# jiang-wenxiang/NeRFail

Hardware: AMD Instinct MI355X
Metric: rays/sec (higher is better)
Workload: dtype f32

## Files before the change

include/nerfail_hip.h:

```cpp
#ifndef NERFAIL_HIP_H
#define NERFAIL_HIP_H

#include <stddef.h>
#include <stdint.h>

#ifdef __cplusplus
extern "C" {
#endif

#define NERFAIL_ABI_VERSION 11

#define NERFAIL_OK 0
#define NERFAIL_EINVAL 1
#define NERFAIL_EHIP 2
#define NERFAIL_ENODEV 3

#define NERFAIL_RAY_FLOATS 11
#define NERFAIL_KNN 8
#define NERFAIL_MAX_DEPTH 16

int nerfail_abi_version(void);
const char* nerfail_last_error(void);
int nerfail_device_name(char* buf_host, size_t buf_len);


int nerfail_get_rays(int H, int W, const float* K4_host, const float* c2w_host,
                     float* rays_o, float* rays_d, void* stream);

int nerfail_pack_rays(const float* rays_o, const float* rays_d, int64_t n, float near_, float far_,
                      float* rays, void* stream);

int nerfail_ray_gen(int H, int W, const float* K4_host, const float* c2w_host, float near_, float far_,
                    int64_t pix_begin, int64_t pix_count, float* rays, void* stream);


int nerfail_sample_coarse(const float* rays, int64_t n_rays, const float* t_vals, int n_samples,
                          const float* t_rand, int lindisp, float* z_vals, float* pts, void* stream);

int nerfail_sample_pdf(const float* bins, const float* weights, int64_t n_rays, int n_bins,
                       const float* u, int u_is_row, int n_samples, float* samples, void* stream);

int nerfail_sample_fine(const float* rays, int64_t n_rays, const float* z_coarse, const float* weights,
                        int n_coarse, const float* u, int u_is_row, int n_fine,
                        float* z_samples, float* z_fine, float* pts, float* z_std, void* stream);


int nerfail_embed(const float* x, int64_t M, int multires, float* out, void* stream);

typedef struct nerfail_mlp_params {
    int32_t D, W;
    int32_t input_ch;
    int32_t input_ch_views;
    int32_t skip;
    int32_t reserved;
    const float* pts_w[NERFAIL_MAX_DEPTH];
    const float* pts_b[NERFAIL_MAX_DEPTH];
    const float* views_w;  const float* views_b;
    const float* feature_w; const float* feature_b;
    const float* alpha_w;  const float* alpha_b;
    const float* rgb_w;    const float* rgb_b;
} nerfail_mlp_params;

size_t nerfail_mlp_packed_floats(int D, int W, int skip);
int nerfail_mlp_pack(const nerfail_mlp_params* params_host, float* packed, void* stream);

int nerfail_mlp_fwd(const float* packed, int D, int W, int skip, const float* pts, const float* viewdirs,
                    int64_t M, int samples_per_ray, float* raw, void* stream);

int nerfail_mlp_fwd_select(int which);

int nerfail_mlp_bwd_select(int which);

int nerfail_mlp_fwd_embedded(const float* packed, int D, int W, int skip, const float* x, int64_t M,
                             float* raw, void* stream);

size_t nerfail_mlp_packed_x3_bytes(int D, int W, int skip);
int nerfail_mlp_pack_x3(const float* packed, int D, int W, int skip, void* x3, void* stream);
int nerfail_mlp_fwd_x3(const float* packed, const void* x3, int D, int W, int skip, const float* pts, const float* viewdirs,
                       int64_t M, int samples_per_ray, float* raw, void* stream);
int nerfail_mlp_fwd_embedded_x3(const float* packed, const void* x3, int D, int W, int skip, const float* x, int64_t M,
                                float* raw, void* stream);
int nerfail_mlp_fwd_rays_x3(const float* packed, const void* x3, int D, int W, int skip, const float* rays,
                            const float* z_vals, int64_t n_rays, int samples_per_ray, float* raw, float* acts, void* stream);

size_t nerfail_mlp_f16_image_bytes(int D, int W, int skip);
int nerfail_mlp_pack_f16(const nerfail_mlp_params* params_host, void* image, void* stream);
int nerfail_mlp_fwd_f16(const float* packed, const void* image, int D, int W, int skip, const float* pts,
                        const float* viewdirs, int64_t M, int samples_per_ray, float* raw, void* stream);
int nerfail_mlp_fwd_f16_train(const float* packed, const void* image, int D, int W, int skip, const float* pts,
                              const float* viewdirs, int64_t M, int samples_per_ray, float* raw, float* acts,
                              void* stream);

size_t nerfail_mlp_f16_image_T_bytes(int D, int W, int skip);
int nerfail_mlp_pack_f16_T(const nerfail_mlp_params* params_host, void* imageT, void* stream);
int nerfail_mlp_bwd_data_f16(const float* packed, const void* imageT, int D, int W, int skip, const float* d_raw,
                             const float* acts, int64_t M, float* dz, void* stream);


size_t nerfail_mlp_train_acts_floats(int D, int W, int64_t M);
size_t nerfail_mlp_train_dz_floats(int D, int W, int64_t M);
int nerfail_mlp_fwd_train(const float* packed, int D, int W, int skip, const float* pts, const float* viewdirs,
                          int64_t M, int samples_per_ray, float* raw, float* acts, void* stream);
int nerfail_mlp_fwd_rays(const float* packed, int D, int W, int skip, const float* rays, const float* z_vals,
                         int64_t n_rays, int samples_per_ray, float* raw, float* acts, void* stream);
size_t nerfail_mlp_packed_T_floats(int D, int W, int skip);
int nerfail_mlp_pack_T(const nerfail_mlp_params* params_host, float* packedT, void* stream);
int nerfail_mlp_pack_train(const nerfail_mlp_params* params_host, float* packed, float* packedT, void* stream);
int nerfail_mlp_bwd_data(const float* packed, const float* packedT, int D, int W, int skip, const float* d_raw,
                         const float* acts, int64_t M, float* dz, void* stream);
int nerfail_mlp_bwd_data2(const float* packed0, const float* packedT0, int64_t M0, const float* packed1,
                          const float* packedT1, int64_t M1, int D, int W, int skip, const float* d_raw,
                          const float* acts, float* dz, void* stream);
#define NERFAIL_DW_BF16X3 1
#define NERFAIL_DW_ACCUMULATE 2
size_t nerfail_mlp_bwd_weights_scratch_bytes(int D, int W, int skip, int64_t M0, int64_t M1, int flags);
int nerfail_mlp_bwd_weights(int D, int W, int skip, const float* acts, const float* dz, int64_t M0,
                            const nerfail_mlp_params* grads0, int64_t M1, const nerfail_mlp_params* grads1, int flags,
                            void* scratch, size_t scratch_bytes, void* stream);


int nerfail_composite(const float* raw, const float* z_vals, const float* rays, const float* noise,
                      int64_t n_rays, int n_samples, int white_bkgd,
                      float* rgb_map, float* disp_map, float* acc_map, float* weights, float* depth_map,
                      const float* pts, float* pts_max, void* stream);

int nerfail_composite_select(int which);

int nerfail_composite_bwd(const float* raw, const float* z_vals, const float* rays, const float* noise,
                          int64_t n_rays, int n_samples, int white_bkgd, const float* g_rgb_map,
                          const float* g_disp_map, const float* g_acc_map, const float* g_depth_map,
                          const float* g_weights, float* d_raw, void* stream);


int nerfail_knn8(const float* queries, int64_t n_queries, const float* points, int64_t n_points,
                 float* dist, float* idx_f32, int32_t* idx_i32, void* stream);

size_t nerfail_knn8_grid_workspace_bytes(int64_t n_points);
int nerfail_knn8_grid(const float* queries, int64_t n_queries, const float* points, int64_t n_points,
                      float* dist, float* idx_f32, int32_t* idx_i32, void* workspace, size_t workspace_bytes,
                      void* stream);
int nerfail_knn8_grid_build(const float* points, int64_t n_points, void* workspace, size_t workspace_bytes, void* stream);
int nerfail_knn8_grid_search(const float* queries, int64_t n_queries, int64_t n_points, float* dist, float* idx_f32,
                             int32_t* idx_i32, const void* workspace, size_t workspace_bytes, void* stream);
int nerfail_knn8_grid_search_view(const float* queries, int height, int width, int64_t n_points, float* dist, float* idx_f32,
                                  int32_t* idx_i32, const void* workspace, size_t workspace_bytes, void* stream);
int nerfail_knn8_grid_stats(unsigned long long* stats);


int nerfail_gauss_weight(const float* dist_and_index, int64_t B, int64_t P, float c, float* out, void* stream);

int nerfail_gauss_compose(const float* ori_img, const float* r, int64_t n_pixels, float* x_rgba, void* stream);

int nerfail_gauss_fwd(const float* spatial, int64_t Ns, const float* weight_and_index, const float* ori_img,
                      int64_t B, int64_t P, float epsilon, float* x, float* x_rgba, float* eps_minmax,
                      void* stream);

typedef struct nerfail_view_fwd {
    const float* weight_and_index;
    const void* ori_img;
} nerfail_view_fwd;
int nerfail_gauss_fwd_views(const float* spatial, int64_t Ns, const nerfail_view_fwd* views, int n_views, int64_t P,
                            int ori_is_u8, float epsilon, float* x, float* x_rgba, float* aux_alpha, unsigned char* aux_mask,
                            float* eps_minmax, void* stream);

int nerfail_gauss_bwd(const float* weight_and_index, const float* ori_img, const float* x,
                      const float* grad_x, const float* grad_x_rgba, int64_t Ns, int64_t B, int64_t P,
                      float epsilon, float* grad_spatial, void* stream);

int nerfail_fingerprint(const void* data, int64_t words_per_item, int64_t n_items, uint64_t* out, void* stream);
size_t nerfail_gauss_csr_workspace_bytes(int64_t Ns, int64_t B, int64_t P);
int nerfail_gauss_csr_build(const float* weight_and_index, int64_t Ns, int64_t B, int64_t P, int32_t* row_ptr,
                            int32_t* contrib, float* w_sorted, int32_t* row_of, void* workspace, size_t workspace_bytes,
                            void* stream);
size_t nerfail_gauss_bwd_scratch_floats(int64_t B, int64_t P, int n_rhs);
int nerfail_gauss_bwd_csr(const float* ori_img, const float* x, const float* grad_x, const float* grad_x_rgba,
                          const int32_t* row_ptr, const int32_t* contrib, const float* w_sorted, const int32_t* row_of,
                          int64_t Ns, int64_t B, int64_t P, float epsilon, float* scratch, int accumulate,
                          float* grad_spatial, void* stream);

size_t nerfail_gauss_view_pack_workspace_bytes(int64_t Ns);
int64_t nerfail_gauss_view_chunks(int64_t n_entries);
int nerfail_gauss_view_pack(const int32_t* row_ptr, const int32_t* row_of, const int32_t* contrib, int64_t Ns,
                            int64_t entry_capacity, int32_t* pos, int32_t* packed, int32_t* chunk_ord, int32_t* n_rows,
                            void* workspace, size_t workspace_bytes, void* stream);

typedef struct nerfail_view_index {
    const int32_t* packed;
    const float* w_sorted;
    const int32_t* chunk_ord;
    const int32_t* pos;
    int64_t n_entries;
    int64_t n_rows;
} nerfail_view_index;
size_t nerfail_gauss_bwd_views_scratch_floats(const nerfail_view_index* views, int n_views, int64_t P, int n_rhs);
int nerfail_gauss_bwd_views(const float* ori_img, const float* x, const float* grad_x, const float* grad_x_rgba,
                            const nerfail_view_index* views, int n_views, int64_t Ns, int64_t P, float epsilon,
                            float* scratch, float* grad_spatial, void* stream);
int nerfail_gauss_bwd_views_rgb(const float* aux_alpha, const unsigned char* aux_mask, const float* grad_x_rgba,
                                const nerfail_view_index* views, int n_views, int64_t Ns, int64_t P, float* scratch,
                                float* grad_rgb, void* stream);
int nerfail_gauss_bwd_views_rgb_step(const float* aux_alpha, const unsigned char* aux_mask, const float* grad_x_rgba,
                                     const nerfail_view_index* views, int n_views, int64_t Ns, int64_t P, float* scratch,
                                     float* grad_rgb, const float* spatial, const float* spatial_init, float a, float epsilon,
                                     int targeted, float* spatial_out, void* stream);
int nerfail_gauss_bwd_view_multi(const float* ori_img, const float* x, const float* grad_x_rgba, int n_rhs,
                                 const nerfail_view_index* view, int64_t Ns, int64_t P, float epsilon, float* scratch,
                                 float* grad_spatial, void* stream);

int nerfail_gauss_bwd_csr_multi(const float* ori_img, const float* x, const float* grad_x_rgba, int n_rhs,
                                const int32_t* row_ptr, const int32_t* contrib, const float* w_sorted, const int32_t* row_of,
                                int64_t Ns, int64_t B, int64_t P, float epsilon, float* scratch, float* grad_spatial,
                                void* stream);

size_t nerfail_deepfool_norms_scratch_bytes(int n_rhs, int64_t n);
int nerfail_deepfool_norms(const float* grads, int n_rhs, int64_t n, void* scratch, size_t scratch_bytes, float* norms2,
                           void* stream);
int nerfail_deepfool_apply(const float* grads, int n_rhs, int64_t n, const int32_t* best, const float* scale,
                           float overshoot, const float* spatial_init, float* rot, float* spatial_out, void* stream);

int nerfail_igsm_step(const float* spatial, const float* grad, const float* spatial_init, int64_t n,
                      float a, float epsilon, int targeted, float* out, void* stream);
int nerfail_igsm_step_rgb(const float* spatial, const float* grad_rgb, const float* spatial_init, int64_t n, float a,
                          float epsilon, int targeted, float* out, void* stream);

typedef struct nerfail_adam_tensor {
    float* param;
    const float* grad;
    float* exp_avg;
    float* exp_avg_sq;
    int64_t numel;
    float step_size;
    float bias_correction2_sqrt;
} nerfail_adam_tensor;
int nerfail_adam_step(const nerfail_adam_tensor* tensors, int n_tensors, double beta1, double beta2, double eps,
                      void* stream);

int nerfail_mse(const float* x, const float* y, int64_t n, float* loss, float* dx, void* stream);


size_t nerfail_cnn_packed_floats(int num_classes);
int nerfail_cnn_pack(const float* const* params_host, int num_classes, float* packed, void* stream);
size_t nerfail_cnn_workspace_bytes(int B, int H, int W, int num_classes);
size_t nerfail_cnn_mask_bytes(int B, int H, int W);
size_t nerfail_cnn_bwd_scratch_bytes(int B, int H, int W);
int nerfail_cnn_fwd(const float* packed, int num_classes, const float* x, int B, int H, int W, float* workspace,
                    unsigned char* masks, float* logits, void* stream);
int nerfail_cnn_bwd_data(const float* packed, int num_classes, const float* workspace, const unsigned char* masks,
                         const float* d_logits, int B, int H, int W, float* scratch, float* d_x, void* stream);

size_t nerfail_cnn_bwd_multi_scratch_bytes(int R, int B, int H, int W);
int nerfail_cnn_bwd_data_multi(const float* packed, int num_classes, const float* workspace, const unsigned char* masks,
                               const float* d_logits , int R, int B, int H, int W, float* scratch,
                               float* d_x , void* stream);

size_t nerfail_cnn_grad_floats(int num_classes);
size_t nerfail_cnn_bwd_weights_scratch_bytes(int B, int H, int W, int num_classes);
int nerfail_cnn_bwd_weights(const float* packed, int num_classes, const float* x, const float* workspace,
                            const unsigned char* masks, const float* d_logits, int B, int H, int W, float* scratch,
                            float* d_params, float* d_x , void* stream);

#ifdef __cplusplus
}
#endif
#endif
```

nerfail_amd/_lib.py:

```python
import ctypes
import os

import torch

_HERE = os.path.dirname(os.path.abspath(__file__))
LIB_PATH = os.environ.get('NERFAIL_HIP_LIB') or os.path.join(_HERE, 'lib', 'libnerfail_hip.so')

ABI_VERSION = 11
MAX_DEPTH = 16
DW_BF16X3, DW_ACCUMULATE = 1, 2
RAY_FLOATS = 11

c_f = ctypes.c_float
c_i = ctypes.c_int
c_i64 = ctypes.c_int64
c_p = ctypes.c_void_p


class NerfailError(RuntimeError):
    """A libnerfail_hip call returned a NERFAIL_E* code."""


class MlpParams(ctypes.Structure):
    _fields_ = [('D', ctypes.c_int32), ('W', ctypes.c_int32), ('input_ch', ctypes.c_int32),
                ('input_ch_views', ctypes.c_int32), ('skip', ctypes.c_int32), ('reserved', ctypes.c_int32),
                ('pts_w', c_p * MAX_DEPTH), ('pts_b', c_p * MAX_DEPTH),
                ('views_w', c_p), ('views_b', c_p), ('feature_w', c_p), ('feature_b', c_p),
                ('alpha_w', c_p), ('alpha_b', c_p), ('rgb_w', c_p), ('rgb_b', c_p)]


SIGNATURES = {
    'nerfail_abi_version': (c_i, []),
    'nerfail_last_error': (ctypes.c_char_p, []),
    'nerfail_device_name': (c_i, [ctypes.c_char_p, ctypes.c_size_t]),
    'nerfail_get_rays': (c_i, [c_i, c_i, c_p, c_p, c_p, c_p, c_p]),
    'nerfail_pack_rays': (c_i, [c_p, c_p, c_i64, c_f, c_f, c_p, c_p]),
    'nerfail_ray_gen': (c_i, [c_i, c_i, c_p, c_p, c_f, c_f, c_i64, c_i64, c_p, c_p]),
    'nerfail_sample_coarse': (c_i, [c_p, c_i64, c_p, c_i, c_p, c_i, c_p, c_p, c_p]),
    'nerfail_sample_pdf': (c_i, [c_p, c_p, c_i64, c_i, c_p, c_i, c_i, c_p, c_p]),
    'nerfail_sample_fine': (c_i, [c_p, c_i64, c_p, c_p, c_i, c_p, c_i, c_i, c_p, c_p, c_p, c_p, c_p]),
    'nerfail_embed': (c_i, [c_p, c_i64, c_i, c_p, c_p]),
    'nerfail_mlp_packed_floats': (ctypes.c_size_t, [c_i, c_i, c_i]),
    'nerfail_mlp_pack': (c_i, [ctypes.POINTER(MlpParams), c_p, c_p]),
    'nerfail_mlp_fwd': (c_i, [c_p, c_i, c_i, c_i, c_p, c_p, c_i64, c_i, c_p, c_p]),
    'nerfail_mlp_fwd_rays': (c_i, [c_p, c_i, c_i, c_i, c_p, c_p, c_i64, c_i, c_p, c_p, c_p]),
    'nerfail_mlp_fwd_select': (c_i, [c_i]),
    'nerfail_mlp_bwd_select': (c_i, [c_i]),
    'nerfail_mlp_fwd_embedded': (c_i, [c_p, c_i, c_i, c_i, c_p, c_i64, c_p, c_p]),
    'nerfail_mlp_packed_x3_bytes': (ctypes.c_size_t, [c_i, c_i, c_i]),
    'nerfail_mlp_pack_x3': (c_i, [c_p, c_i, c_i, c_i, c_p, c_p]),
    'nerfail_mlp_fwd_x3': (c_i, [c_p, c_p, c_i, c_i, c_i, c_p, c_p, c_i64, c_i, c_p, c_p]),
    'nerfail_mlp_fwd_embedded_x3': (c_i, [c_p, c_p, c_i, c_i, c_i, c_p, c_i64, c_p, c_p]),
    'nerfail_mlp_fwd_rays_x3': (c_i, [c_p, c_p, c_i, c_i, c_i, c_p, c_p, c_i64, c_i, c_p, c_p, c_p]),
    'nerfail_mlp_f16_image_bytes': (ctypes.c_size_t, [c_i, c_i, c_i]),
    'nerfail_mlp_pack_f16': (c_i, [ctypes.POINTER(MlpParams), c_p, c_p]),
    'nerfail_mlp_fwd_f16': (c_i, [c_p, c_p, c_i, c_i, c_i, c_p, c_p, c_i64, c_i, c_p, c_p]),
    'nerfail_mlp_fwd_f16_train': (c_i, [c_p, c_p, c_i, c_i, c_i, c_p, c_p, c_i64, c_i, c_p, c_p, c_p]),
    'nerfail_mlp_f16_image_T_bytes': (ctypes.c_size_t, [c_i, c_i, c_i]),
    'nerfail_mlp_pack_f16_T': (c_i, [ctypes.POINTER(MlpParams), c_p, c_p]),
    'nerfail_mlp_bwd_data_f16': (c_i, [c_p, c_p, c_i, c_i, c_i, c_p, c_p, c_i64, c_p, c_p]),
    'nerfail_mlp_train_acts_floats': (ctypes.c_size_t, [c_i, c_i, c_i64]),
    'nerfail_mlp_train_dz_floats': (ctypes.c_size_t, [c_i, c_i, c_i64]),
    'nerfail_mlp_fwd_train': (c_i, [c_p, c_i, c_i, c_i, c_p, c_p, c_i64, c_i, c_p, c_p, c_p]),
    'nerfail_mlp_packed_T_floats': (ctypes.c_size_t, [c_i, c_i, c_i]),
    'nerfail_mlp_pack_T': (c_i, [ctypes.POINTER(MlpParams), c_p, c_p]),
    'nerfail_mlp_pack_train': (c_i, [ctypes.POINTER(MlpParams), c_p, c_p, c_p]),
    'nerfail_mlp_bwd_data': (c_i, [c_p, c_p, c_i, c_i, c_i, c_p, c_p, c_i64, c_p, c_p]),
    'nerfail_mlp_bwd_data2': (c_i, [c_p, c_p, c_i64, c_p, c_p, c_i64, c_i, c_i, c_i, c_p, c_p, c_p, c_p]),
    'nerfail_mlp_bwd_weights_scratch_bytes': (ctypes.c_size_t, [c_i, c_i, c_i, c_i64, c_i64, c_i]),
    'nerfail_mlp_bwd_weights': (c_i, [c_i, c_i, c_i, c_p, c_p, c_i64, ctypes.POINTER(MlpParams), c_i64, ctypes.POINTER(MlpParams),
                                      c_i, c_p, ctypes.c_size_t, c_p]),
    'nerfail_composite': (c_i, [c_p, c_p, c_p, c_p, c_i64, c_i, c_i, c_p, c_p, c_p, c_p, c_p, c_p, c_p, c_p]),
    'nerfail_composite_select': (c_i, [c_i]),
    'nerfail_composite_bwd': (c_i, [c_p, c_p, c_p, c_p, c_i64, c_i, c_i, c_p, c_p, c_p, c_p, c_p, c_p, c_p]),
    'nerfail_knn8': (c_i, [c_p, c_i64, c_p, c_i64, c_p, c_p, c_p, c_p]),
    'nerfail_knn8_grid_workspace_bytes': (ctypes.c_size_t, [c_i64]),
    'nerfail_knn8_grid': (c_i, [c_p, c_i64, c_p, c_i64, c_p, c_p, c_p, c_p, ctypes.c_size_t, c_p]),
    'nerfail_knn8_grid_build': (c_i, [c_p, c_i64, c_p, ctypes.c_size_t, c_p]),
    'nerfail_knn8_grid_stats': (c_i, [c_p]),
    'nerfail_knn8_grid_search': (c_i, [c_p, c_i64, c_i64, c_p, c_p, c_p, c_p, ctypes.c_size_t, c_p]),
    'nerfail_knn8_grid_search_view': (c_i, [c_p, c_i, c_i, c_i64, c_p, c_p, c_p, c_p, ctypes.c_size_t, c_p]),
    'nerfail_gauss_weight': (c_i, [c_p, c_i64, c_i64, c_f, c_p, c_p]),
    'nerfail_gauss_compose': (c_i, [c_p, c_p, c_i64, c_p, c_p]),
    'nerfail_gauss_fwd': (c_i, [c_p, c_i64, c_p, c_p, c_i64, c_i64, c_f, c_p, c_p, c_p, c_p]),
    'nerfail_gauss_bwd': (c_i, [c_p, c_p, c_p, c_p, c_p, c_i64, c_i64, c_i64, c_f, c_p, c_p]),
    'nerfail_gauss_fwd_views': (c_i, [c_p, c_i64, c_p, c_i, c_i64, c_i, c_f, c_p, c_p, c_p, c_p, c_p, c_p]),
    'nerfail_gauss_bwd_views_rgb': (c_i, [c_p, c_p, c_p, c_p, c_i, c_i64, c_i64, c_p, c_p, c_p]),
    'nerfail_igsm_step_rgb': (c_i, [c_p, c_p, c_p, c_i64, c_f, c_f, c_i, c_p, c_p]),
    'nerfail_gauss_bwd_views_rgb_step': (c_i, [c_p, c_p, c_p, c_p, c_i, c_i64, c_i64, c_p, c_p, c_p, c_p, c_f, c_f, c_i, c_p, c_p]),
    'nerfail_fingerprint': (c_i, [c_p, c_i64, c_i64, c_p, c_p]),
    'nerfail_gauss_csr_workspace_bytes': (ctypes.c_size_t, [c_i64, c_i64, c_i64]),
    'nerfail_gauss_csr_build': (c_i, [c_p, c_i64, c_i64, c_i64, c_p, c_p, c_p, c_p, c_p, ctypes.c_size_t, c_p]),
    'nerfail_gauss_bwd_scratch_floats': (ctypes.c_size_t, [c_i64, c_i64, c_i]),
    'nerfail_gauss_view_pack_workspace_bytes': (ctypes.c_size_t, [c_i64]),
    'nerfail_gauss_view_chunks': (c_i64, [c_i64]),
    'nerfail_gauss_view_pack': (c_i, [c_p, c_p, c_p, c_i64, c_i64, c_p, c_p, c_p, c_p, c_p, ctypes.c_size_t, c_p]),
    'nerfail_gauss_bwd_view_multi': (c_i, [c_p, c_p, c_p, c_i, c_p, c_i64, c_i64, c_f, c_p, c_p, c_p]),
    'nerfail_gauss_bwd_views_scratch_floats': (ctypes.c_size_t, [c_p, c_i, c_i64, c_i]),
    'nerfail_gauss_bwd_csr': (c_i, [c_p, c_p, c_p, c_p, c_p, c_p, c_p, c_p, c_i64, c_i64, c_i64, c_f, c_p, c_i, c_p, c_p]),
    'nerfail_gauss_bwd_views': (c_i, [c_p, c_p, c_p, c_p, c_p, c_i, c_i64, c_i64, c_f, c_p, c_p, c_p]),
    'nerfail_gauss_bwd_csr_multi': (c_i, [c_p, c_p, c_p, c_i, c_p, c_p, c_p, c_p, c_i64, c_i64, c_i64, c_f, c_p, c_p, c_p]),
    'nerfail_deepfool_norms_scratch_bytes': (ctypes.c_size_t, [c_i, c_i64]),
    'nerfail_deepfool_norms': (c_i, [c_p, c_i, c_i64, c_p, ctypes.c_size_t, c_p, c_p]),
    'nerfail_deepfool_apply': (c_i, [c_p, c_i, c_i64, c_p, c_p, c_f, c_p, c_p, c_p, c_p]),
    'nerfail_igsm_step': (c_i, [c_p, c_p, c_p, c_i64, c_f, c_f, c_i, c_p, c_p]),
    'nerfail_adam_step': (c_i, [c_p, c_i, ctypes.c_double, ctypes.c_double, ctypes.c_double, c_p]),
    'nerfail_mse': (c_i, [c_p, c_p, c_i64, c_p, c_p, c_p]),
    'nerfail_cnn_packed_floats': (ctypes.c_size_t, [c_i]),
    'nerfail_cnn_pack': (c_i, [c_p, c_i, c_p, c_p]),
    'nerfail_cnn_workspace_bytes': (ctypes.c_size_t, [c_i, c_i, c_i, c_i]),
    'nerfail_cnn_mask_bytes': (ctypes.c_size_t, [c_i, c_i, c_i]),
    'nerfail_cnn_bwd_scratch_bytes': (ctypes.c_size_t, [c_i, c_i, c_i]),
    'nerfail_cnn_fwd': (c_i, [c_p, c_i, c_p, c_i, c_i, c_i, c_p, c_p, c_p, c_p]),
    'nerfail_cnn_bwd_data': (c_i, [c_p, c_i, c_p, c_p, c_p, c_i, c_i, c_i, c_p, c_p, c_p]),
    'nerfail_cnn_bwd_multi_scratch_bytes': (ctypes.c_size_t, [c_i, c_i, c_i, c_i]),
    'nerfail_cnn_bwd_data_multi': (c_i, [c_p, c_i, c_p, c_p, c_p, c_i, c_i, c_i, c_i, c_p, c_p, c_p]),
    'nerfail_cnn_grad_floats': (ctypes.c_size_t, [c_i]),
    'nerfail_cnn_bwd_weights_scratch_bytes': (ctypes.c_size_t, [c_i, c_i, c_i, c_i]),
    'nerfail_cnn_bwd_weights': (c_i, [c_p, c_i, c_p, c_p, c_p, c_p, c_i, c_i, c_i, c_p, c_p, c_p, c_p]),
}



class ViewIndexStruct(ctypes.Structure):
    _fields_ = [('packed', c_p), ('w_sorted', c_p), ('chunk_ord', c_p), ('pos', c_p), ('n_entries', c_i64), ('n_rows', c_i64)]


class ViewFwdStruct(ctypes.Structure):
    _fields_ = [('weight_and_index', c_p), ('ori_img', c_p)]


class AdamTensor(ctypes.Structure):
    _fields_ = [('param', c_p), ('grad', c_p), ('exp_avg', c_p), ('exp_avg_sq', c_p), ('numel', c_i64),
                ('step_size', c_f), ('bias_correction2_sqrt', c_f)]


_lib = None


def load():
    global _lib
    if _lib is not None:
        return _lib
    if not os.path.exists(LIB_PATH):
        raise RuntimeError('nerfail_amd: %s is missing - build it with `python -m nerfail_amd.build` '
                           '(hipcc, gfx950). There is no CPU fallback.' % LIB_PATH)
    lib = ctypes.CDLL(LIB_PATH)
    for name, (res, args) in SIGNATURES.items():
        fn = getattr(lib, name)
        fn.restype = res
        fn.argtypes = args
    v = lib.nerfail_abi_version()
    if v != ABI_VERSION:
        raise RuntimeError('nerfail_amd: ABI version %d, expected %d - rebuild the library' % (v, ABI_VERSION))
    _lib = lib
    return lib


def check(rc):
    if rc != 0:
        msg = load().nerfail_last_error().decode('utf-8', 'replace')
        raise NerfailError('libnerfail_hip error %d: %s' % (rc, msg))


def dev(t, name='tensor'):
    if t is None:
        return None
    if not isinstance(t, torch.Tensor):
        raise TypeError('%s must be a torch.Tensor' % name)
    if not t.is_cuda:
        raise RuntimeError('%s is on %s: nerfail_amd runs on the MI355X only (no CPU path)' % (name, t.device))
    if t.dtype not in (torch.float32, torch.int32, torch.uint8, torch.int64):
        raise TypeError('%s must be float32 (got %s)' % (name, t.dtype))
    if not t.is_contiguous():
        raise ValueError('%s must be contiguous' % name)
    return c_p(t.data_ptr())


def host_floats(values):
    arr = (c_f * len(values))(*[float(v) for v in values])
    return arr


def stream():
    return c_p(torch.cuda.current_stream().cuda_stream)


def f32c(t, device=None):
    t = t.detach()
    if device is not None and t.device != device:
        t = t.to(device)
    if t.dtype != torch.float32:
        t = t.float()
    return t.contiguous()


def device_name():
    buf = ctypes.create_string_buffer(256)
    check(load().nerfail_device_name(buf, 256))
    return buf.value.decode()
```

nerfail_amd/csrc/mlp.hip:

```cpp
#include <stdlib.h>
#include "mlp_layout.h"

namespace nerfail {

bool mlp_x3_covers(const MlpLayout& L, int W);
size_t mlp_x3_bytes(const MlpLayout& L, int W);
int pack_mlp_x3(const float* packed, const MlpLayout& L, int W, void* out, hipStream_t s);
int launch_mlp_x3(const MlpArgs& a, const void* img, int W, hipStream_t s);

template <int NT, bool TRAIN>
__global__ __launch_bounds__(256, 1) void nerf_mlp_fwd_kernel(MlpArgs a) {
    constexpr int OTV = NT / 2;
    const int lane = threadIdx.x & 63;
    const int wave = __builtin_amdgcn_readfirstlane(threadIdx.x >> 6);
    const int h = lane >> 5, j = lane & 31;
    const float* __restrict__ P = a.packed;
    const MlpLayout& L = a.lay;
    const long ntiles = (a.M + 31) / 32;
    const long nrounds = (ntiles + (long)gridDim.x * 4 - 1) / ((long)gridDim.x * 4);

    for (long rnd = 0; rnd < nrounds; ++rnd) {
        const long tile = (rnd * gridDim.x + blockIdx.x) * 4 + wave;
        if (tile >= ntiles) break;
        const long sraw = tile * 32 + j;
        const long s = sraw < a.M ? sraw : a.M - 1;

        float emb[4 * kEmbQuads], demb[4 * kDirQuads];
        encode_sample(a, s, h, emb, demb);

        f32x16 act[NT], acc[NT];
        float* __restrict__ A = nullptr;
        if (TRAIN) {
            A = a.acts + (size_t)tile * (train_a_slots(L.D, NT) * 1024);
            store_enc<10, 4 * kEmbQuads>(A, emb, lane);
            store_enc<4, 4 * kDirQuads>(A + 2 * 1024, demb, lane);
        }
        load_bias<NT>(acc, P + L.b_off[0], h);
        mfma_scalars<NT, kEmbQuads>(acc, P + L.w_off[0], lane, emb);
        relu_to<NT>(act, acc, true);
        if (TRAIN) {
            store_tiles<NT>(A + 3 * 1024, act, lane);
            store_mask<NT>(A + train_mask_slot0(L.D, NT) * 1024, 0, mask_of<NT>(act), lane);
        }

        float alpha = 0.f;
#pragma unroll 1
        for (int l = 1; l <= L.D; ++l) {
            if (l == L.D) {
                const float* wa = P + L.alpha_off;
                float sacc = 0.f;
#pragma unroll
                for (int t = 0; t < NT; ++t) {
                    const f32x4* p = reinterpret_cast<const f32x4*>(wa + (t * 2 + h) * 16);
#pragma unroll
                    for (int r4 = 0; r4 < 4; ++r4) {
                        const f32x4 wv = p[r4];
#pragma unroll
                        for (int e = 0; e < 4; ++e) sacc = fmaf(wv[e], act[t][4 * r4 + e], sacc);
                    }
                }
                sacc += __shfl_xor(sacc, 32, 64);
                alpha = sacc + wa[NT * 32];
            }
            load_bias<NT>(acc, P + L.b_off[l], h);
            const float* w = P + L.w_off[l];
            if (l == L.skip + 1 && L.skip >= 0) {
                if (TRAIN) {
                    float e2[4 * kEmbQuads];
                    load_enc<10, 4 * kEmbQuads>(A, e2, lane);
                    mfma_scalars<NT, kEmbQuads>(acc, w, lane, e2);
                } else {
                    mfma_scalars<NT, kEmbQuads>(acc, w, lane, emb);
                }
                w += kEmbQuads * NT * 256;
            }
            mfma_acts<NT, NT>(acc, w, lane, act);
            relu_to<NT>(act, acc, l < L.D);
            if (TRAIN) {
                store_tiles<NT>(A + (3 + l * NT) * 1024, act, lane);
                if (l < L.D) store_mask<NT>(A + train_mask_slot0(L.D, NT) * 1024, l, mask_of<NT>(act), lane);
            }
        }

        f32x16 hv[OTV];
        load_bias<OTV>(hv, P + L.b_off[L.D + 1], h);
        mfma_acts<OTV, NT>(hv, P + L.w_off[L.D + 1], lane, act);
        if (TRAIN) {
            float d2[4 * kDirQuads];
            load_enc<4, 4 * kDirQuads>(A + 2 * 1024, d2, lane);
            mfma_scalars<OTV, kDirQuads>(hv, P + L.w_off[L.D + 1] + NT * 4 * OTV * 256, lane, d2);
        } else {
            mfma_scalars<OTV, kDirQuads>(hv, P + L.w_off[L.D + 1] + NT * 4 * OTV * 256, lane, demb);
        }
        if (TRAIN) {
            f32x16 hvr[OTV];
            relu_to<OTV>(hvr, hv, true);
            store_tiles<OTV>(A + (3 + (L.D + 1) * NT) * 1024, hvr, lane);
            store_mask<OTV>(A + train_mask_slot0(L.D, NT) * 1024, L.D, mask_of<OTV>(hvr), lane);
        }

        const float* wr = P + L.rgb_off;
        float rgb[3];
#pragma unroll
        for (int c = 0; c < 3; ++c) {
            float sacc = 0.f;
#pragma unroll
            for (int t = 0; t < OTV; ++t) {
                const f32x4* p = reinterpret_cast<const f32x4*>(wr + ((c * OTV + t) * 2 + h) * 16);
#pragma unroll
                for (int r4 = 0; r4 < 4; ++r4) {
                    const f32x4 wv = p[r4];
#pragma unroll
                    for (int e = 0; e < 4; ++e) sacc = fmaf(wv[e], fmaxf(hv[t][4 * r4 + e], 0.f), sacc);
                }
            }
            sacc += __shfl_xor(sacc, 32, 64);
            rgb[c] = sacc + wr[3 * OTV * 32 + c];
        }
        if (h == 0 && sraw < a.M)
            reinterpret_cast<float4*>(a.raw)[sraw] = make_float4(rgb[0], rgb[1], rgb[2], alpha);
    }
}

static int g_fwd_select = [] {
    const char* e = getenv("NERFAIL_FWD_KERNEL");
    return e ? (e[0] == 'r' ? 1 : (e[0] == 'l' ? 2 : (e[0] == 'x' ? 3 : 0))) : 0;
}();
static bool use_lds_kernel(const MlpArgs& a) {
    if (g_fwd_select == 1) return false;
    if (g_fwd_select == 2) return true;
    return !(a.lay.D & 1) && a.lay.D <= 8;
}

static int launch_mlp(const MlpArgs& a, int W, hipStream_t s) {
    if (use_lds_kernel(a)) return launch_mlp_lds(a, W, s);
    const dim3 grid(mlp_grid_blocks((a.M + 31) / 32)), block(256);
    const bool train = a.acts != nullptr;
    switch (W) {
        case 256: if (train) nerf_mlp_fwd_kernel<8, true><<<grid, block, 0, s>>>(a); else nerf_mlp_fwd_kernel<8, false><<<grid, block, 0, s>>>(a); break;
        case 128: if (train) nerf_mlp_fwd_kernel<4, true><<<grid, block, 0, s>>>(a); else nerf_mlp_fwd_kernel<4, false><<<grid, block, 0, s>>>(a); break;
        case 64: if (train) nerf_mlp_fwd_kernel<2, true><<<grid, block, 0, s>>>(a); else nerf_mlp_fwd_kernel<2, false><<<grid, block, 0, s>>>(a); break;
        default: set_error("nerfail_mlp_fwd: unsupported W"); return NERFAIL_EINVAL;
    }
    NF_LAUNCHED("nerf_mlp_fwd_kernel");
    return NERFAIL_OK;
}

static int launch_mlp_x3_or(const MlpArgs& a, const void* img, int W, hipStream_t s) {
    if (a.acts == nullptr && (g_fwd_select == 0 || g_fwd_select == 3)) {
        if (g_fwd_select == 3 || (img != nullptr && mlp_x3_covers(a.lay, W))) {
            if (img == nullptr) { set_error("nerfail_mlp_fwd_x3: NERFAIL_FWD_KERNEL=x without a bf16x3 image"); return NERFAIL_EINVAL; }
            return launch_mlp_x3(a, img, W, s);
        }
    }
    return launch_mlp(a, W, s);
}

}

using namespace nerfail;

extern "C" int nerfail_mlp_fwd_select(int which) {
    const int prev = g_fwd_select;
    if (which >= 0 && which <= 3) g_fwd_select = which;
    return prev;
}

enum MlpInput { kInPts, kInEmbedded, kInRays };
#define MLP_REQUIRE(cond, msg) do { if (!(cond)) { set_error("%s: %s", fn, msg); return NERFAIL_EINVAL; } } while (0)
static int mlp_fwd_entry(const char* fn, MlpInput form, const float* packed, bool use_x3, const void* x3, int D, int W, int skip,
                         const float* in0, const float* in1, int64_t M, int spr, float* raw, float* acts, bool need_acts, void* stream) {
    MLP_REQUIRE(M >= 0, form == kInRays ? "n_rays is negative" : "M is negative");
    MLP_REQUIRE(form == kInEmbedded || spr >= 1, "samples_per_ray must be positive");
    MlpArgs a;
    MLP_REQUIRE(make_layout(D, W, skip, a.lay), "unsupported (D, W)");
    if (form == kInRays) M *= spr;
    if (M == 0) return NERFAIL_OK;
    MLP_REQUIRE(packed != nullptr && in0 != nullptr && (form == kInEmbedded || in1 != nullptr) && raw != nullptr &&
                (!need_acts || acts != nullptr), "NULL pointer");
    a.packed = packed; a.raw = raw; a.acts = acts; a.M = M; a.spr = form == kInEmbedded ? 1 : spr;
    a.pts = form == kInPts ? in0 : nullptr; a.viewdirs = form == kInPts ? in1 : nullptr;
    a.xemb = form == kInEmbedded ? in0 : nullptr;
    a.rays = form == kInRays ? in0 : nullptr; a.z = form == kInRays ? in1 : nullptr;
    return use_x3 ? launch_mlp_x3_or(a, x3, W, as_stream(stream)) : launch_mlp(a, W, as_stream(stream));
}
#undef MLP_REQUIRE

extern "C" int nerfail_mlp_fwd(const float* packed, int D, int W, int skip, const float* pts, const float* viewdirs,
                               int64_t M, int samples_per_ray, float* raw, void* stream) {
    return mlp_fwd_entry(__func__, kInPts, packed, false, nullptr, D, W, skip, pts, viewdirs, M, samples_per_ray, raw, nullptr, false, stream);
}

extern "C" int nerfail_mlp_fwd_embedded(const float* packed, int D, int W, int skip, const float* x, int64_t M, float* raw,
                                        void* stream) {
    return mlp_fwd_entry(__func__, kInEmbedded, packed, false, nullptr, D, W, skip, x, nullptr, M, 1, raw, nullptr, false, stream);
}

extern "C" size_t nerfail_mlp_train_acts_floats(int D, int W, int64_t M) {
    MlpLayout L;
    if (!make_layout(D, W, -1, L) || M < 0) return 0;
    return (size_t)((M + 31) / 32) * make_train_layout(D, W).a_slots * 1024;
}

extern "C" int nerfail_mlp_fwd_train(const float* packed, int D, int W, int skip, const float* pts, const float* viewdirs,
                                     int64_t M, int samples_per_ray, float* raw, float* acts, void* stream) {
    return mlp_fwd_entry(__func__, kInPts, packed, false, nullptr, D, W, skip, pts, viewdirs, M, samples_per_ray, raw, acts, true, stream);
}

extern "C" int nerfail_mlp_fwd_rays(const float* packed, int D, int W, int skip, const float* rays, const float* z_vals,
                                    int64_t n_rays, int samples_per_ray, float* raw, float* acts, void* stream) {
    return mlp_fwd_entry(__func__, kInRays, packed, false, nullptr, D, W, skip, rays, z_vals, n_rays, samples_per_ray, raw, acts, false, stream);
}

extern "C" size_t nerfail_mlp_packed_x3_bytes(int D, int W, int skip) {
    MlpLayout L;
    return make_layout(D, W, skip, L) ? mlp_x3_bytes(L, W) : 0;
}

extern "C" int nerfail_mlp_pack_x3(const float* packed, int D, int W, int skip, void* out, void* stream) {
    MlpLayout L;
    NF_REQUIRE(make_layout(D, W, skip, L), "unsupported (D, W)");
    NF_REQUIRE(packed != nullptr && out != nullptr, "NULL pointer");
    return pack_mlp_x3(packed, L, W, out, as_stream(stream));
}

extern "C" int nerfail_mlp_fwd_x3(const float* packed, const void* x3, int D, int W, int skip, const float* pts,
                                  const float* viewdirs, int64_t M, int samples_per_ray, float* raw, void* stream) {
    return mlp_fwd_entry(__func__, kInPts, packed, true, x3, D, W, skip, pts, viewdirs, M, samples_per_ray, raw, nullptr, false, stream);
}

extern "C" int nerfail_mlp_fwd_embedded_x3(const float* packed, const void* x3, int D, int W, int skip, const float* x, int64_t M,
                                           float* raw, void* stream) {
    return mlp_fwd_entry(__func__, kInEmbedded, packed, true, x3, D, W, skip, x, nullptr, M, 1, raw, nullptr, false, stream);
}

extern "C" int nerfail_mlp_fwd_rays_x3(const float* packed, const void* x3, int D, int W, int skip, const float* rays,
                                       const float* z_vals, int64_t n_rays, int samples_per_ray, float* raw, float* acts, void* stream) {
    return mlp_fwd_entry(__func__, kInRays, packed, true, x3, D, W, skip, rays, z_vals, n_rays, samples_per_ray, raw, acts, false, stream);
}
```

nerfail_amd/csrc/mlp_layout.h:

```cpp
#pragma once
#include "common.h"

namespace nerfail {

typedef float f32x16 __attribute__((ext_vector_type(16)));
typedef float f32x4 __attribute__((ext_vector_type(4)));

constexpr int kPtsCh = 63, kDirCh = 27;
constexpr int kEmbQuads = 8;
constexpr int kDirQuads = 4;

__host__ __device__ inline int enc_channel(int s, int h, int bands) {
    if (s < 3 * bands) return 3 + 6 * (s / 3) + 3 * h + (s % 3);
    if (s == 3 * bands) return h;
    if (s == 3 * bands + 1) return h ? -1 : 2;
    return -1;
}
__host__ __device__ inline int acc_channel(int r, int h) { return (r & 3) + 8 * (r >> 2) + 4 * h; }

__host__ __device__ inline int hidden_channel(int s, int h) { return 32 * (s / 16) + acc_channel(s % 16, h); }
__host__ __device__ inline int weight_column(int emb0, int h0, int dir0, int NT, int s, int h) {
    if (emb0 >= 0) {
        if (s < 4 * kEmbQuads) { const int c = enc_channel(s, h, 10); return c < 0 ? -1 : emb0 + c; }
        s -= 4 * kEmbQuads;
    }
    if (h0 >= 0) {
        if (s < 16 * NT) return h0 + hidden_channel(s, h);
        s -= 16 * NT;
    }
    if (dir0 >= 0) { const int c = enc_channel(s, h, 4); return c < 0 ? -1 : dir0 + c; }
    return -1;
}

struct MlpLayout {
    int NT, D, skip;
    unsigned w_off[NERFAIL_MAX_DEPTH + 2];
    unsigned b_off[NERFAIL_MAX_DEPTH + 2];
    unsigned w_count[NERFAIL_MAX_DEPTH + 2];
    unsigned alpha_off, rgb_off, total;
    unsigned w_total;
    unsigned stream_pad;
};
constexpr int kPiece = 256;

static inline bool layer_has_emb(int l, int skip) { return l == 0 || (skip >= 0 && l == skip + 1); }

static bool make_layout(int D, int W, int skip, MlpLayout& L) {
    if (!(W == 64 || W == 128 || W == 256)) return false;
    if (D < 2 || D > NERFAIL_MAX_DEPTH) return false;
    if (skip >= D - 1) skip = -1;
    L.NT = W / 32; L.D = D; L.skip = skip;
    const int NT = L.NT, OTV = NT / 2;
    unsigned off = 0;
    for (int l = 0; l <= D + 1; ++l) {
        const int OT = (l == D + 1) ? OTV : NT;
        int quads = 0;
        if (l <= D - 1 && layer_has_emb(l, skip)) quads += kEmbQuads;
        if (l > 0) quads += NT * 4;
        if (l == D + 1) quads += kDirQuads;
        L.w_off[l] = off; L.w_count[l] = (unsigned)quads * OT * 256; off += L.w_count[l];
    }
    const unsigned group = 4u * NT * kPiece;
    const unsigned pad = (group - off % group) % group;
    L.stream_pad = pad / kPiece; off += pad; L.w_total = off;
    for (int l = 0; l <= D + 1; ++l) { L.b_off[l] = off; off += kPiece; }
    auto up = [](unsigned n) { return (n + kPiece - 1) / kPiece * kPiece; };
    L.alpha_off = off; off += up((unsigned)NT * 32 + 4);
    L.rgb_off = off; off += up(3u * OTV * 32 + 4);
    L.total = off;
    return true;
}

struct MlpLayerDesc { const float* w; const float* b; int out_f, in_f, OT, emb0, h0, dir0; };
static inline MlpLayerDesc mlp_layer(const nerfail_mlp_params* p, const MlpLayout& L, int l) {
    const int W = 32 * L.NT;
    MlpLayerDesc d = {p->feature_w, p->feature_b, W, W, L.NT, -1, 0, -1};
    if (l < L.D) {
        const bool emb = layer_has_emb(l, L.skip);
        d.w = p->pts_w[l]; d.b = p->pts_b[l];
        d.emb0 = emb ? 0 : -1;
        d.h0 = l == 0 ? -1 : (emb ? kPtsCh : 0);
        d.in_f = (emb ? kPtsCh : 0) + (l == 0 ? 0 : W);
    } else if (l == L.D + 1) {
        d.w = p->views_w; d.b = p->views_b; d.out_f = W / 2; d.in_f = W + kDirCh; d.OT = L.NT / 2; d.dir0 = W;
    }
    return d;
}
static inline const char* mlp_layer_null_msg(const MlpLayout& L, int l) {
    return l < L.D ? "pts_linears pointer is NULL" : (l == L.D ? "feature_linear pointer is NULL" : "views_linears pointer is NULL");
}

inline int mlp_cu_count() {
    static int cus = 0;
    if (cus == 0) {
        int dev = 0, v = 0;
        if (hipGetDevice(&dev) == hipSuccess &&
            hipDeviceGetAttribute(&v, hipDeviceAttributeMultiprocessorCount, dev) == hipSuccess && v > 0) cus = v;
        else cus = 256;
    }
    return cus;
}
inline unsigned mlp_grid_blocks(long ntiles) {
    const long blocks = (ntiles + 3) / 4;
    return (unsigned)(blocks > mlp_cu_count() ? mlp_cu_count() : blocks);
}

__host__ __device__ inline int train_mask_slots(int D) { return (D + 1 + 3) / 4; }
__host__ __device__ inline int train_mask_slot0(int D, int NT) { return 3 + (D + 1) * NT + NT / 2; }
__host__ __device__ inline int train_a_slots(int D, int NT) { return train_mask_slot0(D, NT) + train_mask_slots(D); }

struct TrainLayout {
    int NT, D, OTV;
    int a_slots, a_E, a_V, a_H1, a_F, a_HV, a_MASK;
    int z_slots, z_Z0, z_ZF, z_ZV, z_ZR;
};
static inline TrainLayout make_train_layout(int D, int W) {
    TrainLayout t;
    t.NT = W / 32; t.D = D; t.OTV = t.NT / 2;
    t.a_E = 0; t.a_V = 2; t.a_H1 = 3; t.a_F = 3 + D * t.NT; t.a_HV = t.a_F + t.NT; t.a_MASK = t.a_HV + t.OTV; t.a_slots = t.a_MASK + train_mask_slots(D);
    t.z_Z0 = 0; t.z_ZF = D * t.NT; t.z_ZV = t.z_ZF + t.NT; t.z_ZR = t.z_ZV + t.OTV; t.z_slots = t.z_ZR + 1;
    return t;
}

struct MlpArgs {
    const float* packed;
    const float* pts;
    const float* viewdirs;
    const float* xemb;
    const float* rays;
    const float* z;
    float* raw;
    float* acts;
    long M;
    int spr;
    MlpLayout lay;
};
int launch_mlp_lds(const MlpArgs& a, int W, hipStream_t s);

__device__ __forceinline__ void encode_sample(const MlpArgs& a, long s, int h, float (&emb)[4 * kEmbQuads], float (&demb)[4 * kDirQuads]) {
    if (a.xemb == nullptr) {
        float px[3], vx[3];
        if (a.rays != nullptr) {
            const float* ray = a.rays + NERFAIL_RAY_FLOATS * (s / a.spr);
            const float zz = a.z[s];
#pragma unroll
            for (int d = 0; d < 3; ++d) { px[d] = mul_add_rn(ray[3 + d], zz, ray[d]); vx[d] = ray[8 + d]; }
        } else {
            const float* vd = a.viewdirs + 3 * (s / a.spr);
#pragma unroll
            for (int d = 0; d < 3; ++d) { px[d] = a.pts[3 * s + d]; vx[d] = vd[d]; }
        }
#pragma unroll
        for (int d = 0; d < 3; ++d) {
            const SinCosBands sc(px[d]);
#pragma unroll
            for (int f = 0; f < 10; ++f) emb[3 * f + d] = sc.band_sel(f, h);
        }
        emb[30] = h ? px[1] : px[0];
        emb[31] = h ? 0.f : px[2];
#pragma unroll
        for (int d = 0; d < 3; ++d) {
            const SinCosBands sc(vx[d]);
#pragma unroll
            for (int f = 0; f < 4; ++f) demb[3 * f + d] = sc.band_sel(f, h);
        }
        demb[12] = h ? vx[1] : vx[0];
        demb[13] = h ? 0.f : vx[2];
        demb[14] = 0.f; demb[15] = 0.f;
    } else {
        const float* x = a.xemb + (kPtsCh + kDirCh) * s;
#pragma unroll
        for (int st = 0; st < 4 * kEmbQuads; ++st) {
            const int c = enc_channel(st, h, 10);
            emb[st] = c >= 0 ? x[c] : 0.f;
        }
#pragma unroll
        for (int st = 0; st < 4 * kDirQuads; ++st) {
            const int c = enc_channel(st, h, 4);
            demb[st] = c >= 0 ? x[kPtsCh + c] : 0.f;
        }
    }
}

struct MlpLayoutT {
    unsigned w_off[NERFAIL_MAX_DEPTH + 2];
    unsigned total;
};
static inline void make_layout_T(int D, int NT, MlpLayoutT& L) {
    unsigned off = 0;
    L.w_off[0] = 0;
    for (int l = D + 1; l >= 1; --l) {
        L.w_off[l] = off;
        const int quads = (l == D + 1) ? (NT / 2) * 4 : NT * 4;
        off += (unsigned)quads * NT * 256;
    }
    L.total = off;
}

struct BwdArgs {
    const float* packed;
    const float* packedT;
    const float* packed2;
    const float* packedT2;
    long split;
    const float* d_raw;
    const float* acts;
    float* dz;
    long M;
    int blocks0;
    MlpLayout lay;
    MlpLayoutT layT;
    TrainLayout tl;
};
int launch_bwd_data_lds(const BwdArgs& a, int W, hipStream_t s);

template <int OT>
__device__ __forceinline__ void load_bias(f32x16 (&acc)[OT], const float* __restrict__ b, int h) {
#pragma unroll
    for (int t = 0; t < OT; ++t) {
        const f32x4* p = reinterpret_cast<const f32x4*>(b + (t * 2 + h) * 16);
        const f32x4 v0 = p[0], v1 = p[1], v2 = p[2], v3 = p[3];
        acc[t] = (f32x16){v0[0], v0[1], v0[2], v0[3], v1[0], v1[1], v1[2], v1[3],
                          v2[0], v2[1], v2[2], v2[3], v3[0], v3[1], v3[2], v3[3]};
    }
}

constexpr int kPrefetchQuads = 1;
template <int OT, int NQ, int PFQ = kPrefetchQuads, typename BSel>
__device__ __forceinline__ void mfma_part(f32x16 (&acc)[OT], const float* __restrict__ w, int lane, BSel bsel) {
    const f32x4* wp = reinterpret_cast<const f32x4*>(w) + lane;
    constexpr int PF = PFQ < NQ ? PFQ : (NQ > 1 ? NQ - 1 : 1), RING = PF + 1;
    f32x4 ring[RING][OT];
#pragma unroll
    for (int p = 0; p < PF && p < NQ; ++p)
#pragma unroll
        for (int t = 0; t < OT; ++t) ring[p][t] = wp[(p * OT + t) * 64];
#pragma unroll
    for (int q = 0; q < NQ; ++q) {
        if (q + PF < NQ) {
#pragma unroll
            for (int t = 0; t < OT; ++t)
                ring[(q + PF) % RING][t] = wp[((q + PF) * OT + t) * 64];
            __builtin_amdgcn_sched_barrier(0);
        }
#pragma unroll
        for (int e = 0; e < 4; ++e)
#pragma unroll
            for (int t = 0; t < OT; ++t)
                acc[t] = __builtin_amdgcn_mfma_f32_32x32x2f32(ring[q % RING][t][e], bsel(q, e), acc[t], 0, 0, 0);
        if (q + PF < NQ) __builtin_amdgcn_sched_barrier(0);
    }
}

template <int OT, int NQ, int PFQ = kPrefetchQuads>
__device__ __forceinline__ void mfma_scalars(f32x16 (&acc)[OT], const float* __restrict__ w, int lane,
                                             const float (&bsrc)[4 * NQ]) {
    mfma_part<OT, NQ, PFQ>(acc, w, lane, [&](int q, int e) { return bsrc[4 * q + e]; });
}

template <int OT, int NT, int PFQ = kPrefetchQuads>
__device__ __forceinline__ void mfma_acts(f32x16 (&acc)[OT], const float* __restrict__ w, int lane,
                                          const f32x16 (&in)[NT]) {
    mfma_part<OT, NT * 4, PFQ>(acc, w, lane, [&](int q, int e) { return in[q >> 2][4 * (q & 3) + e]; });
}

template <int NT>
__device__ __forceinline__ void relu_to(f32x16 (&dst)[NT], const f32x16 (&src)[NT], bool relu) {
#pragma unroll
    for (int t = 0; t < NT; ++t)
#pragma unroll
        for (int r = 0; r < 16; ++r) dst[t][r] = relu ? fmaxf(src[t][r], 0.f) : src[t][r];
}

__device__ __forceinline__ int slot_pos(int j) { return (j >> 4) * 512 + (j & 15); }
constexpr int kSlotCh = 16;

__device__ __forceinline__ int acc_lane_off(int lane) { return slot_pos(lane & 31) + (lane >> 5) * 4 * kSlotCh; }
__device__ __forceinline__ constexpr int acc_reg_off(int r) { return ((r & 3) + 8 * (r >> 2)) * kSlotCh; }

__device__ __forceinline__ void slot_store(float* p, float v) {
    __builtin_nontemporal_store(v, p);
}
template <int NTILES>
__device__ __forceinline__ void store_tiles(float* __restrict__ base, const f32x16 (&a)[NTILES], int lane) {
    float* __restrict__ lp = base + acc_lane_off(lane);
#pragma unroll
    for (int t = 0; t < NTILES; ++t)
#pragma unroll
        for (int r = 0; r < 16; ++r) slot_store(lp + t * 1024 + acc_reg_off(r), a[t][r]);
}
__device__ __forceinline__ f32x16 load_tile(const float* __restrict__ base, int lane) {
    const float* __restrict__ lp = base + acc_lane_off(lane);
    f32x16 v;
#pragma unroll
    for (int r = 0; r < 16; ++r) v[r] = lp[acc_reg_off(r)];
    return v;
}
template <int NTILES>
struct TileMask { unsigned w[(NTILES + 1) / 2]; };

__device__ __forceinline__ unsigned relu_bit(float a) {
    unsigned b;
    asm("v_med3_i32 %0, %1, 0, 1" : "=v"(b) : "v"(a));
    return b;
}
template <int NTILES>
__device__ __forceinline__ TileMask<NTILES> mask_of(const f32x16 (&a)[NTILES]) {
    TileMask<NTILES> m;
#pragma unroll
    for (int i = 0; i < (NTILES + 1) / 2; ++i) m.w[i] = 0u;
#pragma unroll
    for (int t = 0; t < NTILES; ++t)
#pragma unroll
        for (int r = 0; r < 16; ++r) m.w[t >> 1] |= relu_bit(a[t][r]) << (16 * (t & 1) + r);
    return m;
}
template <int NTILES>
__device__ __forceinline__ void store_mask(float* __restrict__ mask_slots, int entry, const TileMask<NTILES>& m, int lane) {
    unsigned* __restrict__ q = reinterpret_cast<unsigned*>(mask_slots) + entry * 256 + lane * 4;
    if constexpr (NTILES == 8) {
        *reinterpret_cast<uint4*>(q) = make_uint4(m.w[0], m.w[1], m.w[2], m.w[3]);
    } else {
#pragma unroll
        for (int i = 0; i < (NTILES + 1) / 2; ++i) q[i] = m.w[i];
    }
}
template <int NTILES>
__device__ __forceinline__ TileMask<NTILES> load_mask(const float* __restrict__ mask_slots, int entry, int lane) {
    const unsigned* __restrict__ q = reinterpret_cast<const unsigned*>(mask_slots) + entry * 256 + lane * 4;
    TileMask<NTILES> m;
    if constexpr (NTILES == 8) {
        const uint4 v = *reinterpret_cast<const uint4*>(q);
        m.w[0] = v.x; m.w[1] = v.y; m.w[2] = v.z; m.w[3] = v.w;
    } else {
#pragma unroll
        for (int i = 0; i < (NTILES + 1) / 2; ++i) m.w[i] = q[i];
    }
    return m;
}
template <int NTILES>
__device__ __forceinline__ float mask_apply(const TileMask<NTILES>& m, int t, int r, float x) {
    const int k = __builtin_amdgcn_sbfe((int)m.w[t >> 1], 16 * (t & 1) + r, 1);
    return __uint_as_float(__float_as_uint(x) & (unsigned)k);
}

__device__ __forceinline__ constexpr int enc_ch_off(int c) { return (c >> 5) * 1024 + (c & 31) * kSlotCh; }

template <int BANDS, int NSTEPS>
__device__ __forceinline__ void store_enc(float* __restrict__ base, const float (&e)[NSTEPS], int lane) {
    const int h = lane >> 5, j = lane & 31;
    float* __restrict__ lpz = base + slot_pos(j);
    float* __restrict__ lp3 = lpz + h * 3 * kSlotCh;
    float* __restrict__ lpx = lpz + (h ? enc_ch_off(32) : enc_ch_off(29));
#pragma unroll
    for (int s = 0; s < 3 * BANDS; ++s) {
        const int c0 = 3 + 6 * (s / 3) + (s % 3);
        if (c0 == 29) lpx[0] = e[s];
        else lp3[enc_ch_off(c0)] = e[s];
    }
    lpz[h * kSlotCh] = e[3 * BANDS];
    constexpr int nch = 3 + 6 * BANDS, cap = ((nch + 31) / 32) * 32;
    if (h == 0) lpz[2 * kSlotCh] = e[3 * BANDS + 1];
#pragma unroll
    for (int c = nch; c < cap; ++c)
        if (((c - nch) & 1) == h) lpz[enc_ch_off(c)] = 0.f;
}
template <int BANDS, int NSTEPS>
__device__ __forceinline__ void load_enc(const float* __restrict__ base, float (&e)[NSTEPS], int lane) {
    const int h = lane >> 5, j = lane & 31;
    const float* __restrict__ lpz = base + slot_pos(j);
    const float* __restrict__ lp3 = lpz + h * 3 * kSlotCh;
    const float* __restrict__ lpx = lpz + (h ? enc_ch_off(32) : enc_ch_off(29));
#pragma unroll
    for (int s = 0; s < 3 * BANDS; ++s) {
        const int c0 = 3 + 6 * (s / 3) + (s % 3);
        e[s] = (c0 == 29) ? lpx[0] : lp3[enc_ch_off(c0)];
    }
    e[3 * BANDS] = lpz[h * kSlotCh];
    const float z = lpz[2 * kSlotCh];
    e[3 * BANDS + 1] = h ? 0.f : z;
#pragma unroll
    for (int s = 3 * BANDS + 2; s < NSTEPS; ++s) e[s] = 0.f;
}

}
```

nerfail_amd/csrc/mlp_x3.hip:

```cpp
#include "mlp_lds.h"

namespace nerfail {

typedef __bf16 bf16x8 __attribute__((ext_vector_type(8)));
typedef __bf16 bf16x2 __attribute__((ext_vector_type(2)));
typedef unsigned u32x4 __attribute__((ext_vector_type(4)));
typedef float f32x2 __attribute__((ext_vector_type(2)));
typedef __attribute__((address_space(3))) const u32x4 lds_cu4;
typedef __attribute__((address_space(3))) const f32x2 lds_cf2;

struct X3Cfg {
    static constexpr int NT = 8;
    static constexpr int OT = 2 * NT;
    static constexpr int GP = 24;
    static constexpr int S = 4;
    static constexpr int RP = GP * S;
    static constexpr int GPW = GP / 4;
    static constexpr int SPG = GP / 3;
    static constexpr int kSync = SPG - 2;
    static constexpr int kMaxDepth = 8;
    static constexpr int kAlphaFloats = (NT * 32 + 4 + kPiece - 1) / kPiece * kPiece;
    static constexpr int kRgbFloats = (3 * (NT / 2) * 32 + 4 + kPiece - 1) / kPiece * kPiece;
    static constexpr int kConstMax = (kMaxDepth + 2) * kPiece + kAlphaFloats + kRgbFloats;
    static constexpr int kParkQuads = kEmbQuads + kDirQuads;
    static constexpr int kParkFloats = 4 * 64 * 4 * kParkQuads;
    static_assert((S - 2) * GPW <= 63, "vmcnt is a 6-bit counter");
    static_assert(GPW <= 8, "dma() covers 8 pieces per wave and group");
};

struct X3Layout {
    unsigned off[NERFAIL_MAX_DEPTH + 2];
    unsigned pieces;
};
static inline bool make_x3_layout(const MlpLayout& L, int W, X3Layout& X) {
    if (W != 256 || (L.D & 1) || L.D > X3Cfg::kMaxDepth) return false;
    unsigned off = 0;
    for (int l = 0; l <= L.D + 1; ++l) {
        const unsigned OT = (l == L.D + 1) ? L.NT / 2 : L.NT;
        const unsigned quads = L.w_count[l] / (OT * kPiece);
        if (quads & 3) return false;
        X.off[l] = off;
        off += quads / 4 * (2 * OT) * 3;
    }
    X.pieces = off;
    return off % X3Cfg::GP == 0;
}

__device__ __forceinline__ unsigned cvt_bf2(float x0, float x1) {
    return __builtin_bit_cast(unsigned, __builtin_convertvector((f32x2){x0, x1}, bf16x2));
}
__device__ __forceinline__ void sub_bf2(float& x0, float& x1, unsigned p) {
    x0 -= __uint_as_float(p << 16);
    x1 -= __uint_as_float(p & 0xffff0000u);
}

struct X3PackArgs {
    MlpLayout L;
    X3Layout X;
};
__global__ void pack_x3_kernel(const float* __restrict__ packed, X3PackArgs p, u32x4* __restrict__ img) {
    const long g = (long)blockIdx.x * blockDim.x + threadIdx.x;
    const long ts = g >> 6;
    const int lane = (int)(g & 63);
    if (ts * 3 >= p.X.pieces) return;
    int l = 0;
    while (l < p.L.D + 1 && ts * 3 >= p.X.off[l + 1]) ++l;
    const int OT32 = (l == p.L.D + 1) ? p.L.NT / 2 : p.L.NT, OT16 = 2 * OT32;
    const long r = ts - p.X.off[l] / 3;
    const int u = (int)(r / OT16), t = (int)(r % OT16);
    const int row = 16 * t + (lane & 15), lg = lane >> 4;
    const int q = 4 * u + (lg >> 1);
    const float* w = packed + p.L.w_off[l] + (row >> 5) * kPiece + ((row & 31) + 32 * (lg & 1)) * 4;
    const f32x4 q0 = *reinterpret_cast<const f32x4*>(w + (q * OT32) * kPiece);
    const f32x4 q1 = *reinterpret_cast<const f32x4*>(w + ((q + 2) * OT32) * kPiece);
    float x[8] = {q0[0], q0[1], q0[2], q0[3], q1[0], q1[1], q1[2], q1[3]};
    u32x4 hi, mid, lo;
#pragma unroll
    for (int k = 0; k < 4; ++k) {
        float a = x[2 * k], b = x[2 * k + 1];
        hi[k] = cvt_bf2(a, b);
        sub_bf2(a, b, hi[k]);
        mid[k] = cvt_bf2(a, b);
        sub_bf2(a, b, mid[k]);
        lo[k] = cvt_bf2(a, b);
    }
    u32x4* o = img + (p.X.off[l] + (long)r * 3) * 64 + lane;
    o[0] = hi;
    o[64] = mid;
    o[128] = lo;
}

struct X3Ring {
    using C = X3Cfg;
    __amdgpu_buffer_rsrc_t rsrc;
    int voff;
    float* ring;
    const float* rl;
    int total;
    int src, slot, rd, wave;
    u32x4 f1[3], f2[3];

    template <int I>
    __device__ __forceinline__ void dma_at() const {
        constexpr int B4 = I / 4;
        const int first = wave * C::GPW + 4 * B4;
        __builtin_amdgcn_raw_ptr_buffer_load_lds(rsrc, (lds_void_t*)(ring + (slot * C::GP + first) * kPiece), 16, voff,
                                                 (src + first) * (kPiece * 4), (I % 4) * kPiece * 4, 0);
    }
    __device__ __forceinline__ void dma(int i) const {
        switch (i) {
            case 0: dma_at<0>(); break;   case 1: dma_at<1>(); break;   case 2: dma_at<2>(); break;   case 3: dma_at<3>(); break;
            case 4: dma_at<4>(); break;   case 5: dma_at<5>(); break;   case 6: dma_at<6>(); break;   case 7: dma_at<7>(); break;
            default: break;
        }
    }
    __device__ __forceinline__ void group_issued() {
        src += C::GP;
        if (src >= total) src = 0;
        slot = (slot + 1 == C::S) ? 0 : slot + 1;
    }
    __device__ __forceinline__ void boundary() const {
        lds_wait_vmcnt<(C::S - 2) * C::GPW>();
        asm volatile("s_waitcnt lgkmcnt(0)" ::: "memory");
        __builtin_amdgcn_s_barrier();
        asm volatile("" ::: "memory");
    }
    __device__ __forceinline__ u32x4 frag(int POS, int p) const { return *(lds_cu4*)(rl + (rd + 3 * POS + p) * kPiece); }
    __device__ __forceinline__ void next_group() {
        rd += C::GP;
        if (rd >= C::RP) rd = 0;
    }
    __device__ __forceinline__ void start() {
#pragma unroll
        for (int g = 0; g < C::S - 1; ++g) {
#pragma unroll
            for (int i = 0; i < C::GPW; ++i) dma(i);
            group_issued();
        }
        boundary();
        dma(0);
        dma(1);
#pragma unroll
        for (int p = 0; p < 3; ++p) f1[p] = frag(0, p);
#pragma unroll
        for (int p = 0; p < 3; ++p) f2[p] = frag(1, p);
    }
};

__device__ __forceinline__ void mfma_x3(f32x4& acc, const u32x4& a, const u32x4& b) {
    acc = __builtin_amdgcn_mfma_f32_16x16x32_bf16(__builtin_bit_cast(bf16x8, a), __builtin_bit_cast(bf16x8, b), acc, 0, 0, 0);
}

__device__ __forceinline__ int x3_lane_off(int g) { return 16 * (g & 1) + 4 * (g >> 1); }
__device__ __forceinline__ int x3_tile_off(int t) { return 32 * (t >> 1) + 8 * (t & 1); }

template <int OT, int NIN>
__device__ __forceinline__ void x3_head(const f32x4 (&x)[NIN][2], const float* w, float (&out)[2]) {
    float s0 = 0.f, s1 = 0.f;
#pragma unroll
    for (int t = 0; t < OT; ++t) {
        const f32x4 wv = lds_read4(w + x3_tile_off(t));
#pragma unroll
        for (int e = 0; e < 4; ++e) {
            float v0 = x[t][0][e], v1 = x[t][1][e];
            asm("" : "+v"(v0), "+v"(v1));
            s0 = fmaf(wv[e], relu_bits(v0), s0);
            s1 = fmaf(wv[e], relu_bits(v1), s1);
        }
        __builtin_amdgcn_sched_barrier(0);
    }
    s0 += __shfl_xor(s0, 16, 64);
    s1 += __shfl_xor(s1, 16, 64);
    out[0] = s0 + __shfl_xor(s0, 32, 64);
    out[1] = s1 + __shfl_xor(s1, 32, 64);
}
template <int OT, int NIN>
__device__ __forceinline__ void x3_head3(const f32x4 (&x)[NIN][2], const float* w, int stride, float (&out)[2][3]) {
    float s[2][3] = {};
#pragma unroll
    for (int t = 0; t < OT; ++t) {
        const float* p = w + x3_tile_off(t);
        const f32x4 w0 = lds_read4(p), w1 = lds_read4(p + stride), w2 = lds_read4(p + 2 * stride);
#pragma unroll
        for (int e = 0; e < 4; ++e) {
#pragma unroll
            for (int n = 0; n < 2; ++n) {
                float v = x[t][n][e];
                asm("" : "+v"(v));
                v = relu_bits(v);
                s[n][0] = fmaf(w0[e], v, s[n][0]);
                s[n][1] = fmaf(w1[e], v, s[n][1]);
                s[n][2] = fmaf(w2[e], v, s[n][2]);
            }
        }
        __builtin_amdgcn_sched_barrier(0);
    }
#pragma unroll
    for (int n = 0; n < 2; ++n)
#pragma unroll
        for (int c = 0; c < 3; ++c) {
            const float v = s[n][c] + __shfl_xor(s[n][c], 16, 64);
            out[n][c] = v + __shfl_xor(v, 32, 64);
        }
}

template <class Side>
__device__ __forceinline__ void x3_step(X3Ring& st, const int POS, f32x4 (&acc)[2], const u32x4 (&b)[2][3], Side side) {
    using C = X3Cfg;
    const int P = (POS - C::kSync + C::SPG) % C::SPG;
    const int AHEAD = (POS + 2) % C::SPG;
    u32x4 a[3];
#pragma unroll
    for (int p = 0; p < 3; ++p) { a[p] = st.f1[p]; st.f1[p] = st.f2[p]; }
    if (P == 0) st.boundary();
#pragma unroll
    for (int k = 0; k < 12; ++k) {
        const int pr = k >> 1, n = k & 1;
        const int pa = pr == 0 || pr == 4 ? 1 : pr == 2 ? 2 : 0;
        const int pb = pr == 0 || pr == 3 ? 1 : pr == 1 ? 2 : 0;
        __builtin_amdgcn_sched_barrier(0);
        mfma_x3(acc[n], a[pa], b[n][pb]);
        __builtin_amdgcn_sched_barrier(0);
        side(k);
        if (k == 0 && P < C::GPW) st.dma(P);
        if (k == 1) st.f2[1] = st.frag(AHEAD, 1);
        if (k == 2) st.f2[0] = st.frag(AHEAD, 0);
        if (k == 3) {
            st.f2[2] = st.frag(AHEAD, 2);
            if (AHEAD == C::SPG - 1) st.next_group();
        }
    }
    if (P == C::SPG - 1) st.group_issued();
    __builtin_amdgcn_sched_barrier(0);
}

template <int OT, int NS, bool RELU, class Ld, class Hook>
__device__ __forceinline__ void x3_part(X3Ring& st, f32x4 (&out)[X3Cfg::OT][2], Ld ld, Hook hook) {
    static_assert((NS * OT) % X3Cfg::SPG == 0 && OT >= 8, "a part is a whole number of ring groups; 8 pairs per step");
    auto act = [](float v) { return RELU ? relu_bits(v) : v; };
    auto bf2_f32 = [](unsigned q) { return (f32x2){__uint_as_float(q << 16), __uint_as_float(q & 0xffff0000u)}; };
    u32x4 b[2][3];
#pragma unroll
    for (int n = 0; n < 2; ++n)
#pragma unroll
        for (int p = 0; p < 4; ++p) {
            f32x2 x = {act(ld(0, n, p, 0)), act(ld(0, n, p, 1))};
            b[n][0][p] = cvt_bf2(x[0], x[1]);
            x -= bf2_f32(b[n][0][p]);
            b[n][1][p] = cvt_bf2(x[0], x[1]);
            x -= bf2_f32(b[n][1][p]);
            b[n][2][p] = cvt_bf2(x[0], x[1]);
        }
#pragma unroll
    for (int s = 0; s < NS; ++s) {
        u32x4 bn[2][3];
        f32x2 xs[8], es[8];
#pragma unroll
        for (int t = 0; t < OT; ++t) {
            auto side = [&](int k) {
                if (s + 1 < NS && t < 8) {
                    const int n = t >> 2, p = t & 3;
                    if (k == 0) xs[t][0] = ld(s + 1, n, p, 0);
                    if (k == 1) xs[t][1] = ld(s + 1, n, p, 1);
                    if (RELU && k == 2) xs[t][0] = relu_bits(xs[t][0]);
                    if (RELU && k == 3) xs[t][1] = relu_bits(xs[t][1]);
                    if (k == 4) bn[n][0][p] = cvt_bf2(xs[t][0], xs[t][1]);
                    if (k == 5) es[t] = bf2_f32(bn[n][0][p]);
                    if (k == 6) xs[t] -= es[t];
                    if (k == 7) bn[n][1][p] = cvt_bf2(xs[t][0], xs[t][1]);
                    if (k == 8) es[t] = bf2_f32(bn[n][1][p]);
                    if (k == 9) xs[t] -= es[t];
                    if (k == 10) bn[n][2][p] = cvt_bf2(xs[t][0], xs[t][1]);
                }
                if (k >= 10) hook(s, t, k);
            };
            x3_step(st, (s * OT + t) % X3Cfg::SPG, out[t], b, side);
        }
        if (s + 1 < NS) {
#pragma unroll
            for (int n = 0; n < 2; ++n)
#pragma unroll
                for (int p = 0; p < 3; ++p) b[n][p] = bn[n][p];
        }
    }
}

template <int NT, int SKIP>
__global__ __launch_bounds__(256, 1) void nerf_mlp_fwd_x3_kernel(MlpArgs a, const void* img, int img_pieces) {
    static_assert(NT == X3Cfg::NT, "W = 256 only");
    using C = X3Cfg;
    constexpr int OT = C::OT, OTV = OT / 2;
    __shared__ __attribute__((aligned(16))) float smem[C::RP * kPiece + C::kConstMax + C::kParkFloats];
    const int tid = threadIdx.x, lane = tid & 63;
    const int wave = __builtin_amdgcn_readfirstlane(tid >> 6);
    const int h = lane >> 5, j = lane & 31;
    const int g = lane >> 4, c = lane & 15;
    const MlpLayout& L = a.lay;
    float* const ring0 = smem;
    float* const cst = smem + C::RP * kPiece;
    float* const park_w = cst + C::kConstMax + wave * (64 * 4 * C::kParkQuads);
    float* const park = park_w + lane * 4;
    const float* const park_rd = park_w + (c + 32 * (g & 1)) * 4 + (g >> 1) * 256;
    {
        const int n = (int)(L.total - L.b_off[0]);
        const float* __restrict__ gm = a.packed + L.b_off[0];
        for (int i = tid * 4; i < n; i += 1024) *reinterpret_cast<f32x4*>(cst + i) = *reinterpret_cast<const f32x4*>(gm + i);
    }
    __syncthreads();
    const float* const c_alpha = cst + (L.alpha_off - L.b_off[0]);
    const float* const c_rgb = cst + (L.rgb_off - L.b_off[0]);
    int lane_off = x3_lane_off(g);
    asm volatile("" : "+v"(lane_off));
    const float* const cst_g = cst + lane_off;

    X3Ring st;
    st.rsrc = __builtin_amdgcn_make_buffer_rsrc(const_cast<void*>(img), 0, img_pieces * (kPiece * 4), 0x00020000);
    st.voff = lane * 16; st.ring = ring0; st.rl = ring0 + lane * 4;
    st.total = img_pieces; st.src = 0; st.slot = 0; st.rd = 0; st.wave = wave;
    st.start();

    f32x4 P[OT][2], Q[OT][2];
    auto bias_tile = [&](f32x4 (&dst)[OT][2], int l, int i, int t0, int t, int k) {
        if (t == t0 && k == 10) {
            dst[i][0] = lds_read4(cst_g + l * kPiece + x3_tile_off(i));
            asm volatile("" : "+a"(dst[i][0]));
        }
        if (t == t0 + 1 && k == 11) {
            dst[i][1] = dst[i][0];
            asm volatile("" : "+a"(dst[i][1]));
        }
    };
#pragma unroll
    for (int t = 0; t < OT; ++t) { bias_tile(P, 0, t, 0, 0, 10); bias_tile(P, 0, t, 0, 1, 11); }

    const int ntiles = (int)((a.M + 31) / 32);
    const int nrounds = (int)((ntiles + (long)gridDim.x * 4 - 1) / ((long)gridDim.x * 4));
    for (int rnd = 0; rnd < nrounds; ++rnd) {
        const int tile_own = (int)(((long)rnd * gridDim.x + blockIdx.x) * 4 + wave);
        const int tile = tile_own < ntiles ? tile_own : ntiles - 1;
        int jj = j;
        asm volatile("" : "+v"(jj));
        const long sraw = (long)tile * 32 + jj;
        const long s = sraw < a.M ? sraw : a.M - 1;
        {
            float emb[4 * kEmbQuads], demb[4 * kDirQuads];
            int hh = h;
            asm volatile("" : "+v"(hh));
            encode_sample(a, s, hh, emb, demb);
#pragma unroll
            for (int k = 0; k < kEmbQuads; ++k)
                *reinterpret_cast<f32x4*>(park + k * 256) = (f32x4){emb[4 * k], emb[4 * k + 1], emb[4 * k + 2], emb[4 * k + 3]};
#pragma unroll
            for (int k = 0; k < kDirQuads; ++k)
                *reinterpret_cast<f32x4*>(park + (kEmbQuads + k) * 256) =
                    (f32x4){demb[4 * k], demb[4 * k + 1], demb[4 * k + 2], demb[4 * k + 3]};
        }
        auto b_park = [&](int q0) {
            return [=](int u, int n, int p, int e) {
                return *(__attribute__((address_space(3))) const float*)(park_rd + n * 64 + (q0 + 4 * u + 2 * (p >> 1)) * 256 + 2 * (p & 1) + e);
            };
        };
        auto b_acc = [](const f32x4 (&in)[OT][2]) {
            return [&in](int u, int n, int p, int e) { return in[2 * u + (p >> 1)][n][2 * (p & 1) + e]; };
        };
        auto no_hook = [](int, int, int) {};
        x3_part<OT, kEmbQuads / 4, false>(st, P, b_park(0), [&](int u, int t, int k) {
            for (int i = 0; i < 8; ++i) bias_tile(Q, 1, 8 * u + i, 7 + i, t, k);
        });

        float alpha[2] = {0.f, 0.f};
        auto layer = [&](f32x4 (&in)[OT][2], f32x4 (&out)[OT][2], int l, bool may_skip, bool may_be_last) __attribute__((always_inline)) {
            if (may_be_last && l == L.D) {
                x3_head<OT>(in, c_alpha + lane_off, alpha);
                alpha[0] += c_alpha[NT * 32];
                alpha[1] += c_alpha[NT * 32];
            }
            if (may_skip && l == L.skip + 1) x3_part<OT, kEmbQuads / 4, false>(st, out, b_park(0), no_hook);
            x3_part<OT, NT, true>(st, out, b_acc(in), [&](int u, int t, int k) {
                if (u > 0) { bias_tile(in, l + 1, 2 * u - 2, 8, t, k); bias_tile(in, l + 1, 2 * u - 1, 9, t, k); }
                if (u == NT - 1) { bias_tile(in, l + 1, 2 * u, 10, t, k); bias_tile(in, l + 1, 2 * u + 1, 11, t, k); }
            });
        };
#pragma unroll 1
        for (int l = 1; l < L.D; l += 2) {
            layer(P, Q, l, SKIP == 1, false);
            layer(Q, P, l + 1, SKIP == 2, true);
        }
        x3_part<OTV, NT, false>(st, Q, b_acc(P), [&](int u, int t, int k) {
            if (u > 0) { bias_tile(P, 0, 2 * u - 2, 2, t, k); bias_tile(P, 0, 2 * u - 1, 3, t, k); }
            if (u == NT - 1) { bias_tile(P, 0, 2 * u, 4, t, k); bias_tile(P, 0, 2 * u + 1, 5, t, k); }
        });
        x3_part<OTV, kDirQuads / 4, false>(st, Q, b_park(kEmbQuads), no_hook);
        float rgb[2][3];
        x3_head3<OTV>(Q, c_rgb + lane_off, OTV * 16, rgb);
        const int n = g & 1;
        int je = 16 * n + c;
        asm volatile("" : "+v"(je));
        const long sout = (long)tile * 32 + je;
        if (g < 2 && sout < a.M && tile_own < ntiles)
            reinterpret_cast<float4*>(a.raw)[sout] = make_float4((n ? rgb[1][0] : rgb[0][0]) + c_rgb[3 * OTV * 16 + 0],
                                                                 (n ? rgb[1][1] : rgb[0][1]) + c_rgb[3 * OTV * 16 + 1],
                                                                 (n ? rgb[1][2] : rgb[0][2]) + c_rgb[3 * OTV * 16 + 2],
                                                                 n ? alpha[1] : alpha[0]);
    }
    lds_wait_vmcnt<0>();
}

bool mlp_x3_covers(const MlpLayout& L, int W) {
    X3Layout X;
    return make_x3_layout(L, W, X) && L.total - L.b_off[0] <= (unsigned)X3Cfg::kConstMax;
}

size_t mlp_x3_bytes(const MlpLayout& L, int W) {
    X3Layout X;
    return mlp_x3_covers(L, W) && make_x3_layout(L, W, X) ? (size_t)X.pieces * kPiece * 4 : 0;
}

int pack_mlp_x3(const float* packed, const MlpLayout& L, int W, void* out, hipStream_t s) {
    X3PackArgs p;
    p.L = L;
    if (!mlp_x3_covers(L, W) || !make_x3_layout(L, W, p.X)) { set_error("nerfail_mlp_pack_x3: shape not covered (W = 256, even D <= 8)"); return NERFAIL_EINVAL; }
    const long threads = (long)p.X.pieces / 3 * 64;
    pack_x3_kernel<<<dim3((unsigned)((threads + 255) / 256)), dim3(256), 0, s>>>(packed, p, reinterpret_cast<u32x4*>(out));
    NF_LAUNCHED("pack_x3_kernel");
    return NERFAIL_OK;
}

int launch_mlp_x3(const MlpArgs& a, const void* img, int W, hipStream_t s) {
    X3Layout X;
    if (!mlp_x3_covers(a.lay, W) || !make_x3_layout(a.lay, W, X)) { set_error("nerf_mlp_fwd_x3_kernel: shape not covered (W = 256, even D <= 8)"); return NERFAIL_EINVAL; }
    if (a.M >= (1L << 36)) { set_error("nerfail_mlp_fwd: M must be below 2^36 samples per call"); return NERFAIL_EINVAL; }
    const dim3 grid(mlp_grid_blocks((a.M + 31) / 32)), block(256);
    const int skip_layer = a.lay.skip >= 0 ? a.lay.skip + 1 : -1;
    if (skip_layer < 0) nerf_mlp_fwd_x3_kernel<8, 0><<<grid, block, 0, s>>>(a, img, (int)X.pieces);
    else if (skip_layer & 1) nerf_mlp_fwd_x3_kernel<8, 1><<<grid, block, 0, s>>>(a, img, (int)X.pieces);
    else nerf_mlp_fwd_x3_kernel<8, 2><<<grid, block, 0, s>>>(a, img, (int)X.pieces);
    NF_LAUNCHED("nerf_mlp_fwd_x3_kernel");
    return NERFAIL_OK;
}

}
```

nerfail_amd/run_nerf.py:

```python
import os
import time

import numpy as np
import torch

from . import _lib
from .optim import Adam, decayed_lrate
from .run_nerf_helpers import (NeRF, Embedder, get_embedder, get_rays, get_rays_np, img2mse, mse2psnr, to8b,
                               sample_pdf, linspace01, _cuda, _k4, _c2w12)

np.random.seed(0)
DEBUG = False


def batchify(fn, chunk):
    if chunk is None:
        return fn

    def ret(inputs):
        return torch.cat([fn(inputs[i:i + chunk]) for i in range(0, inputs.shape[0], chunk)], 0)
    return ret


def _is_fused(embed_fn, embeddirs_fn, fn):
    return (isinstance(fn, NeRF) and isinstance(embed_fn, Embedder) and embed_fn.multires == 10 and
            isinstance(embeddirs_fn, Embedder) and embeddirs_fn.multires == 4)


def _mlp_points(fn, pts, viewdirs):
    R, N = pts.shape[0], pts.shape[1]
    raw = torch.empty((R, N, 4), dtype=torch.float32, device=pts.device)
    if getattr(fn, 'precision', 'f32') == 'f16x3':
        _lib.check(_lib.load().nerfail_mlp_fwd_f16(_lib.dev(fn.packed()), _lib.dev(fn.packed_f16()), fn.D, fn.W, fn._skip(),
                                                   _lib.dev(pts, 'pts'), _lib.dev(viewdirs, 'viewdirs'), R * N, N,
                                                   _lib.dev(raw), _lib.stream()))
        return raw
    _lib.check(_lib.load().nerfail_mlp_fwd_x3(_lib.dev(fn.packed()), _lib.dev(fn.packed_x3()), fn.D, fn.W, fn._skip(),
                                              _lib.dev(pts, 'pts'), _lib.dev(viewdirs, 'viewdirs'), R * N, N, _lib.dev(raw),
                                              _lib.stream()))
    return raw


def _mlp_rays(fn, rays, z_vals, acts=None):
    R, N = z_vals.shape
    raw = torch.empty((R, N, 4), dtype=torch.float32, device=z_vals.device)
    x3 = fn.packed_x3() if acts is None else None
    _lib.check(_lib.load().nerfail_mlp_fwd_rays_x3(_lib.dev(fn.packed()), _lib.dev(x3), fn.D, fn.W, fn._skip(),
                                                   _lib.dev(rays, 'rays'), _lib.dev(z_vals, 'z_vals'), R, N, _lib.dev(raw),
                                                   _lib.dev(acts), _lib.stream()))
    return raw


def run_network(inputs, viewdirs, fn, embed_fn, embeddirs_fn, netchunk=1024 * 64):
    dev = _cuda()
    inputs = _lib.f32c(inputs, dev)
    if viewdirs is not None and _is_fused(embed_fn, embeddirs_fn, fn) and inputs.dim() == 3:
        return _mlp_points(fn, inputs, _lib.f32c(viewdirs, dev))
    inputs_flat = torch.reshape(inputs, [-1, inputs.shape[-1]])
    embedded = embed_fn(inputs_flat)
    if viewdirs is not None:
        input_dirs = viewdirs[:, None].expand(inputs.shape)
        input_dirs_flat = torch.reshape(input_dirs, [-1, input_dirs.shape[-1]])
        embedded = torch.cat([embedded, embeddirs_fn(input_dirs_flat)], -1)
    outputs_flat = batchify(fn, netchunk)(embedded)
    return torch.reshape(outputs_flat, list(inputs.shape[:-1]) + [outputs_flat.shape[-1]])


class FusedNetworkQuery:

    def __init__(self, embed_fn, embeddirs_fn, netchunk=1024 * 64):
        self.embed_fn, self.embeddirs_fn, self.netchunk = embed_fn, embeddirs_fn, netchunk

    def __call__(self, inputs, viewdirs, network_fn):
        return run_network(inputs, viewdirs, network_fn, embed_fn=self.embed_fn, embeddirs_fn=self.embeddirs_fn,
                           netchunk=self.netchunk)


def batchify_rays(rays_flat, chunk=1024 * 32, **kwargs):
    all_ret = {}
    for i in range(0, rays_flat.shape[0], chunk):
        ret = render_rays(rays_flat[i:i + chunk], **kwargs)
        for k in ret:
            all_ret.setdefault(k, []).append(ret[k])
    return {k: (torch.cat(v, 0) if len(v) > 1 else v[0]) for k, v in all_ret.items()}


def _pack_rays(rays_o, rays_d, near, far):
    dev = _cuda()
    o = _lib.f32c(rays_o, dev).reshape(-1, 3)
    d = _lib.f32c(rays_d, dev).reshape(-1, 3)
    rays = torch.empty((o.shape[0], _lib.RAY_FLOATS), dtype=torch.float32, device=dev)
    _lib.check(_lib.load().nerfail_pack_rays(_lib.dev(o), _lib.dev(d), o.shape[0], float(near), float(far),
                                             _lib.dev(rays), _lib.stream()))
    return rays


def ray_gen(H, W, K, c2w, near, far, pix_begin=0, pix_count=None):
    dev = _cuda()
    n = H * W - pix_begin if pix_count is None else pix_count
    rays = torch.empty((n, _lib.RAY_FLOATS), dtype=torch.float32, device=dev)
    _lib.check(_lib.load().nerfail_ray_gen(int(H), int(W), _k4(K), _c2w12(c2w), float(near), float(far),
                                           int(pix_begin), int(n), _lib.dev(rays), _lib.stream()))
    return rays


def _render(H, W, K, chunk, rays, c2w, ndc, near, far, use_viewdirs, c2w_staticcam, want_pts_max, kwargs):
    if ndc:
        raise NotImplementedError('ndc=True is LLFF-only (RN:112-114); the blender configs pass ndc=False')
    if not use_viewdirs:
        raise NotImplementedError('HIP path implements use_viewdirs=True (all configs/*.txt)')
    if c2w is not None:
        if c2w_staticcam is not None:
            rays_flat = ray_gen(H, W, K, c2w_staticcam, near, far)
            rays_flat[:, 8:11] = ray_gen(H, W, K, c2w, near, far)[:, 8:11]
        else:
            rays_flat = ray_gen(H, W, K, c2w, near, far)
        sh = (H, W, 3)
    else:
        rays_o, rays_d = rays
        sh = tuple(rays_d.shape)
        rays_flat = _pack_rays(rays_o, rays_d, near, far)
    all_ret = batchify_rays(rays_flat, chunk, want_pts_max=want_pts_max, **kwargs)
    for k in all_ret:
        all_ret[k] = torch.reshape(all_ret[k], list(sh[:-1]) + list(all_ret[k].shape[1:]))
    k_extract = ['rgb_map', 'disp_map', 'acc_map'] + (['pts_max'] if want_pts_max else [])
    ret_list = [all_ret[k] for k in k_extract]
    ret_dict = {k: all_ret[k] for k in all_ret if k not in k_extract}
    return ret_list + [ret_dict]


def render(H, W, K, chunk=1024 * 32, rays=None, c2w=None, ndc=True, near=0., far=1., use_viewdirs=False,
           c2w_staticcam=None, **kwargs):
    return _render(H, W, K, chunk, rays, c2w, ndc, near, far, use_viewdirs, c2w_staticcam, False, kwargs)


def render_path(render_poses, hwf, K, chunk, render_kwargs, gt_imgs=None, savedir=None, render_factor=0):
    H, W, focal = hwf
    if render_factor != 0:
        H, W, focal = H // render_factor, W // render_factor, focal / render_factor
    rgbs, disps = [], []
    t = time.time()
    for i, c2w in enumerate(render_poses):
        print(i, time.time() - t)
        t = time.time()
        rgb, disp, acc, _ = render(H, W, K, chunk=chunk, c2w=c2w[:3, :4], **render_kwargs)
        rgbs.append(rgb.cpu().numpy())
        disps.append(disp.cpu().numpy())
        if savedir is not None:
            import imageio
            imageio.imwrite(os.path.join(savedir, '{:03d}.png'.format(i)), to8b(rgbs[-1]))
    return np.stack(rgbs, 0), np.stack(disps, 0)


def create_nerf(args):
    dev = _cuda()
    embed_fn, input_ch = get_embedder(args.multires, args.i_embed)
    input_ch_views, embeddirs_fn = 0, None
    if args.use_viewdirs:
        embeddirs_fn, input_ch_views = get_embedder(args.multires_views, args.i_embed)
    output_ch = 5 if args.N_importance > 0 else 4
    skips = [4]
    model = NeRF(D=args.netdepth, W=args.netwidth, input_ch=input_ch, output_ch=output_ch, skips=skips,
                 input_ch_views=input_ch_views, use_viewdirs=args.use_viewdirs).to(dev)
    grad_vars = list(model.parameters())
    model_fine = None
    if args.N_importance > 0:
        model_fine = NeRF(D=args.netdepth_fine, W=args.netwidth_fine, input_ch=input_ch, output_ch=output_ch,
                          skips=skips, input_ch_views=input_ch_views, use_viewdirs=args.use_viewdirs).to(dev)
        grad_vars += list(model_fine.parameters())
    network_query_fn = FusedNetworkQuery(embed_fn, embeddirs_fn, args.netchunk)
    optimizer = Adam(params=grad_vars, lr=args.lrate, betas=(0.9, 0.999))
    start = 0
    basedir, expname = args.basedir, args.expname
    if getattr(args, 'ft_path', None) is not None and args.ft_path != 'None':
        ckpts = [args.ft_path]
    else:
        d = os.path.join(basedir, expname)
        ckpts = [os.path.join(d, f) for f in sorted(os.listdir(d)) if 'tar' in f] if os.path.isdir(d) else []
    print('Found ckpts', ckpts)
    if len(ckpts) > 0 and not args.no_reload:
        ckpt = torch.load(ckpts[-1], map_location=dev)
        start = ckpt['global_step']
        optimizer.load_state_dict(ckpt['optimizer_state_dict'])
        model.load_state_dict(ckpt['network_fn_state_dict'])
        if model_fine is not None:
            model_fine.load_state_dict(ckpt['network_fine_state_dict'])
    render_kwargs_train = {
        'network_query_fn': network_query_fn, 'perturb': args.perturb, 'N_importance': args.N_importance,
        'network_fine': model_fine, 'N_samples': args.N_samples, 'network_fn': model,
        'use_viewdirs': args.use_viewdirs, 'white_bkgd': args.white_bkgd, 'raw_noise_std': args.raw_noise_std,
    }
    if args.dataset_type != 'llff' or args.no_ndc:
        render_kwargs_train['ndc'] = False
        render_kwargs_train['lindisp'] = args.lindisp
    render_kwargs_test = {k: render_kwargs_train[k] for k in render_kwargs_train}
    render_kwargs_test['perturb'] = False
    render_kwargs_test['raw_noise_std'] = 0.
    return render_kwargs_train, render_kwargs_test, start, grad_vars, optimizer


def _composite(raw, z_vals, rays, noise, white_bkgd, pts=None, want_pts_max=None):
    R, N = z_vals.shape
    dev = raw.device
    if want_pts_max is None:
        want_pts_max = pts is not None
    rgb_map = torch.empty((R, 3), dtype=torch.float32, device=dev)
    disp_map = torch.empty((R,), dtype=torch.float32, device=dev)
    acc_map = torch.empty((R,), dtype=torch.float32, device=dev)
    weights = torch.empty((R, N), dtype=torch.float32, device=dev)
    depth_map = torch.empty((R,), dtype=torch.float32, device=dev)
    pts_max = torch.empty((R, 3), dtype=torch.float32, device=dev) if want_pts_max else None
    _lib.check(_lib.load().nerfail_composite(
        _lib.dev(raw, 'raw'), _lib.dev(z_vals, 'z_vals'), _lib.dev(rays, 'rays'), _lib.dev(noise, 'noise'), R, N,
        int(bool(white_bkgd)), _lib.dev(rgb_map), _lib.dev(disp_map), _lib.dev(acc_map), _lib.dev(weights),
        _lib.dev(depth_map), _lib.dev(pts, 'pts') if want_pts_max else None, _lib.dev(pts_max), _lib.stream()))
    return rgb_map, disp_map, acc_map, weights, depth_map, pts_max


def _noise(shape, raw_noise_std, pytest, noise, dev):
    if noise is not None:
        return _lib.f32c(noise, dev).reshape(shape)
    if raw_noise_std > 0.:
        if pytest:
            np.random.seed(0)
            return torch.Tensor(np.random.rand(*shape) * raw_noise_std).to(dev).contiguous()
        return (torch.randn(shape, device=dev) * raw_noise_std).contiguous()
    return None


def raw2outputs(raw, z_vals, rays_d, raw_noise_std=0, white_bkgd=False, pytest=False, noise=None):
    dev = _cuda()
    raw_in = raw
    raw, z_vals, rays_d = _lib.f32c(raw, dev), _lib.f32c(z_vals, dev), _lib.f32c(rays_d, dev)
    R = z_vals.shape[0]
    rays = torch.zeros((R, _lib.RAY_FLOATS), dtype=torch.float32, device=dev)
    rays[:, 3:6] = rays_d
    nz = _noise(tuple(z_vals.shape), raw_noise_std, pytest, noise, dev)
    if nz is None:
        from . import ops
        raw_g = raw_in.to(dev).float().contiguous() if isinstance(raw_in, torch.Tensor) and raw_in.requires_grad else raw
        return tuple(torch.ops.nerfail_mi.composite(raw_g, z_vals, rays, bool(white_bkgd)))
    return _composite(raw, z_vals, rays, nz, white_bkgd)[:5]


def render_rays(ray_batch, network_fn, network_query_fn, N_samples, retraw=False, lindisp=False, perturb=0.,
                N_importance=0, network_fine=None, white_bkgd=False, raw_noise_std=0., verbose=False, pytest=False,
                want_pts_max=False, t_rand=None, u=None, noise=None, noise_fine=None):
    dev = _cuda()
    rays = _lib.f32c(ray_batch, dev)
    if rays.shape[-1] != _lib.RAY_FLOATS:
        raise NotImplementedError('ray_batch must be [R, 11] (use_viewdirs=True packing, RN:116-123)')
    R = rays.shape[0]
    q = network_query_fn
    fused = q is None or (isinstance(q, FusedNetworkQuery) and _is_fused(q.embed_fn, q.embeddirs_fn, network_fn))

    if perturb > 0. and t_rand is None:
        if pytest:
            np.random.seed(0)
            t_rand = torch.Tensor(np.random.rand(R, N_samples))
        else:
            t_rand = torch.rand((R, N_samples), device=dev)
    t_rand = _lib.f32c(t_rand, dev) if perturb > 0. else None
    if N_importance > 0 and u is None:
        det = (perturb == 0.)
        if pytest:
            np.random.seed(0)
            u = torch.Tensor(np.linspace(0., 1., N_importance)) if det else torch.Tensor(np.random.rand(R, N_importance))
        else:
            u = linspace01(N_importance, dev) if det else torch.rand((R, N_importance), device=dev)
    if u is not None:
        u = _lib.f32c(u, dev)
    nz = _noise((R, N_samples), raw_noise_std, pytest, noise, dev)
    nzf = _noise((R, N_samples + N_importance), raw_noise_std, pytest, noise_fine, dev) if N_importance > 0 else None

    def pipeline(rays, train=False):
        return _render_rays_pipeline(rays, network_fn, network_fine, q if not fused else None, N_samples, N_importance,
                                     lindisp, white_bkgd, t_rand, u, nz, nzf, want_pts_max, train)

    needs_grad = fused and torch.is_grad_enabled() and any(
        p.requires_grad for n in (network_fn, network_fine) if n is not None for p in n.parameters())
    if needs_grad:
        from . import _train
        nets = [network_fn] + ([network_fine] if network_fine is not None else [])
        params = [p for n in nets for p in _train.ordered_params(n)]
        cfg = dict(pipeline=pipeline, network_fn=network_fn, network_fine=network_fine, white_bkgd=white_bkgd,
                   retraw=retraw)
        o = _train.RenderRaysTrain.apply(rays, cfg, *params)
        out = dict(zip(('rgb_map', 'disp_map', 'acc_map', 'rgb0', 'disp0', 'acc0', 'z_std', 'pts_max', 'raw'), o))
    else:
        out = pipeline(rays, False)

    ret = {'rgb_map': out['rgb_map'], 'disp_map': out['disp_map'], 'acc_map': out['acc_map']}
    if want_pts_max:
        ret['pts_max'] = out['pts_max']
    if retraw:
        ret['raw'] = out['raw']
    if N_importance > 0:
        ret.update(rgb0=out['rgb0'], disp0=out['disp0'], acc0=out['acc0'], z_std=out['z_std'])
    if DEBUG:
        for k in ret:
            if torch.isnan(ret[k]).any() or torch.isinf(ret[k]).any():
                print(f"! [Numerical Error] {k} contains nan or inf.")
    return ret


def _render_rays_pipeline(rays, network_fn, network_fine, user_query, N_samples, N_importance, lindisp, white_bkgd,
                          t_rand, u, nz, nzf, want_pts_max, train):
    dev = rays.device
    lib = _lib.load()
    R = rays.shape[0]
    st = _lib.stream()
    viewdirs = rays[:, 8:11].contiguous()

    def empty():
        return torch.empty((0,), dtype=torch.float32, device=dev)

    def wants_pts(fn):
        return user_query is not None or getattr(fn, 'precision', 'f32') == 'f16x3'

    def query(p, z, fn):
        if user_query is not None:
            return _lib.f32c(user_query(p, viewdirs, fn), dev), None
        if train:
            from . import _train
            a_ = acts_for.pop(0) if acts_for else None
            if p is None:
                return _train.mlp_fwd_train_rays(fn, rays, z, acts=a_)
            return _train.mlp_fwd_train(fn, p, viewdirs, acts=a_)
        if p is None:
            return _mlp_rays(fn, rays, z), None
        return _mlp_points(fn, p, viewdirs), None

    acts_all, acts_for = None, []
    if train and user_query is None and N_importance > 0:
        from . import _train
        run_fn_ = network_fn if network_fine is None else network_fine
        if _train._same_arch(network_fn, run_fn_) and (R * N_samples) % 32 == 0:
            nc, nf = _train.acts_floats(network_fn, R * N_samples), _train.acts_floats(run_fn_, R * (N_samples + N_importance))
            acts_all = torch.empty((nc + nf,), dtype=torch.float32, device=dev)
            acts_for = [acts_all[:nc], acts_all[nc:]]

    z_vals = torch.empty((R, N_samples), dtype=torch.float32, device=dev)
    pts = torch.empty((R, N_samples, 3), dtype=torch.float32, device=dev) if wants_pts(network_fn) else None
    t_lin = linspace01(N_samples, dev)
    _lib.check(lib.nerfail_sample_coarse(_lib.dev(rays), R, _lib.dev(t_lin), int(N_samples),
                                         _lib.dev(t_rand, 't_rand'), int(bool(lindisp)), _lib.dev(z_vals), _lib.dev(pts), st))
    raw, acts = query(pts, z_vals, network_fn)
    last_pass = not (N_importance > 0)
    rgb_map, disp_map, acc_map, weights, depth_map, pts_max = _composite(
        raw, z_vals, rays, nz, white_bkgd, pts, want_pts_max and last_pass)
    out = {'rgb0': empty(), 'disp0': empty(), 'acc0': empty(), 'z_std': empty()}
    saved = {'rays': rays, 'coarse': dict(raw=raw, z=z_vals, acts=acts, noise=nz), 'fine': None, 'acts_all': acts_all}
    if N_importance > 0:
        out.update(rgb0=rgb_map, disp0=disp_map, acc0=acc_map)
        Nt = N_samples + N_importance
        z_samples = torch.empty((R, N_importance), dtype=torch.float32, device=dev)
        z_fine = torch.empty((R, Nt), dtype=torch.float32, device=dev)
        run_fn = network_fn if network_fine is None else network_fine
        pts = torch.empty((R, Nt, 3), dtype=torch.float32, device=dev) if wants_pts(run_fn) else None
        z_std = torch.empty((R,), dtype=torch.float32, device=dev)
        _lib.check(lib.nerfail_sample_fine(_lib.dev(rays), R, _lib.dev(z_vals), _lib.dev(weights), int(N_samples),
                                           _lib.dev(u, 'u'), int(u.dim() == 1), int(N_importance), _lib.dev(z_samples),
                                           _lib.dev(z_fine), _lib.dev(pts), _lib.dev(z_std), st))
        z_vals = z_fine
        raw, acts = query(pts, z_vals, run_fn)
        rgb_map, disp_map, acc_map, weights, depth_map, pts_max = _composite(
            raw, z_vals, rays, nzf, white_bkgd, pts, want_pts_max)
        out['z_std'] = z_std
        saved['fine'] = dict(raw=raw, z=z_vals, acts=acts, noise=nzf)
    out.update(rgb_map=rgb_map, disp_map=disp_map, acc_map=acc_map, raw=raw,
               pts_max=pts_max if pts_max is not None else empty())
    if train:
        out['_saved'] = saved
    return out
```

nerfail_amd/run_nerf_helpers.py:

```python
import numpy as np
import torch
import torch.nn as nn

from . import _lib

class _Img2Mse(torch.autograd.Function):

    @staticmethod
    def forward(ctx, x, y):
        xc, yc = _lib.f32c(x), _lib.f32c(y)
        loss = torch.empty((), dtype=torch.float32, device=x.device)
        dx = torch.empty_like(xc) if x.requires_grad else None
        _lib.check(_lib.load().nerfail_mse(_lib.dev(xc), _lib.dev(yc), xc.numel(), _lib.dev(loss), _lib.dev(dx), _lib.stream()))
        ctx.dx = dx
        return loss

    @staticmethod
    def backward(ctx, g):
        return (None if ctx.dx is None else ctx.dx * g), None


MSE_FUSED_MAX = 1 << 16


def img2mse(x, y):
    if (isinstance(x, torch.Tensor) and isinstance(y, torch.Tensor) and x.is_cuda and y.is_cuda and x.dtype == torch.float32
            and y.dtype == torch.float32 and x.shape == y.shape and not y.requires_grad and 0 < x.numel() <= MSE_FUSED_MAX):
        return _Img2Mse.apply(x, y)
    return torch.mean((x - y) ** 2)


mse2psnr = lambda x: -10. * torch.log(x) / torch.log(torch.Tensor([10.]).to(x.device))
to8b = lambda x: (255 * np.clip(x, 0, 1)).astype(np.uint8)


def _cuda():
    if not torch.cuda.is_available():
        raise RuntimeError('nerfail_amd needs an MI355X (torch.cuda.is_available() is False); no CPU path exists')
    return torch.device('cuda', torch.cuda.current_device())


class Embedder:

    def __init__(self, multires):
        self.multires = int(multires)
        self.out_dim = 3 + 6 * self.multires

    def embed(self, inputs):
        x = _lib.f32c(inputs, _cuda())
        assert x.shape[-1] == 3, 'input_dims is 3 (RH:58)'
        flat = x.reshape(-1, 3)
        out = torch.empty((flat.shape[0], self.out_dim), dtype=torch.float32, device=x.device)
        _lib.check(_lib.load().nerfail_embed(_lib.dev(flat, 'inputs'), flat.shape[0], self.multires,
                                             _lib.dev(out), _lib.stream()))
        return out.reshape(x.shape[:-1] + (self.out_dim,))

    __call__ = embed


def get_embedder(multires, i=0, device=None):
    if i == -1:
        return nn.Identity(), 3
    eo = Embedder(multires)
    return eo, eo.out_dim


class NeRF(nn.Module):

    def __init__(self, D=8, W=256, input_ch=3, input_ch_views=3, output_ch=4, skips=[4], use_viewdirs=False):
        super(NeRF, self).__init__()
        self.D = D
        self.W = W
        self.input_ch = input_ch
        self.input_ch_views = input_ch_views
        self.skips = skips
        self.use_viewdirs = use_viewdirs
        self.pts_linears = nn.ModuleList(
            [nn.Linear(input_ch, W)] + [nn.Linear(W, W) if i not in self.skips else nn.Linear(W + input_ch, W)
                                        for i in range(D - 1)])
        self.views_linears = nn.ModuleList([nn.Linear(input_ch_views + W, W // 2)])
        if use_viewdirs:
            self.feature_linear = nn.Linear(W, W)
            self.alpha_linear = nn.Linear(W, 1)
            self.rgb_linear = nn.Linear(W // 2, 3)
        else:
            self.output_linear = nn.Linear(W, output_ch)
        self._packed = None
        self._packed_key = None
        self._packed16 = None
        self._packed16_key = None
        self._packed_x3 = None
        self._packed_x3_key = None
        self.precision = 'f32'

    def _skip(self):
        s = [i for i in self.skips if i < self.D - 1]
        if len(s) > 1:
            raise NotImplementedError('one skip connection supported (the reference always uses skips=[4])')
        return s[0] if s else -1

    def packed(self):
        if not self.use_viewdirs:
            raise NotImplementedError('HIP path implements use_viewdirs=True (all NeRFail configs, configs/*.txt)')
        params = list(self.parameters())
        if not params[0].is_cuda:
            raise RuntimeError('NeRF parameters are on %s: call .cuda() - there is no CPU path' % params[0].device)
        key = tuple((p.data_ptr(), p._version) for p in params)
        if self._packed is not None and key == self._packed_key:
            return self._packed
        lib = _lib.load()
        n = lib.nerfail_mlp_packed_floats(self.D, self.W, self._skip())
        if n == 0:
            raise NotImplementedError('unsupported NeRF shape D=%d W=%d (W in {64,128,256})' % (self.D, self.W))
        keep = []
        mp = self._mlp_params(keep)
        buf = torch.empty((n,), dtype=torch.float32, device=params[0].device)
        _lib.check(lib.nerfail_mlp_pack(mp, _lib.dev(buf), _lib.stream()))
        self._packed, self._packed_key = buf, key
        return buf

    def packed_x3(self):
        f32 = self.packed()
        params = list(self.parameters())
        key = tuple((p.data_ptr(), p._version) for p in params)
        if self._packed_x3_key == key:
            return self._packed_x3
        lib = _lib.load()
        n = lib.nerfail_mlp_packed_x3_bytes(self.D, self.W, self._skip())
        buf = None
        if n:
            buf = torch.empty((n,), dtype=torch.uint8, device=f32.device)
            _lib.check(lib.nerfail_mlp_pack_x3(_lib.dev(f32), self.D, self.W, self._skip(), _lib.dev(buf), _lib.stream()))
        self._packed_x3, self._packed_x3_key = buf, key
        return buf

    def _mlp_params(self, keep):
        mp = _lib.MlpParams()
        mp.D, mp.W, mp.input_ch, mp.input_ch_views, mp.skip = self.D, self.W, self.input_ch, self.input_ch_views, self._skip()

        def ptr(t):
            t = _lib.f32c(t)
            keep.append(t)
            return t.data_ptr()
        for i, l in enumerate(self.pts_linears):
            mp.pts_w[i] = ptr(l.weight)
            mp.pts_b[i] = ptr(l.bias)
        mp.views_w, mp.views_b = ptr(self.views_linears[0].weight), ptr(self.views_linears[0].bias)
        mp.feature_w, mp.feature_b = ptr(self.feature_linear.weight), ptr(self.feature_linear.bias)
        mp.alpha_w, mp.alpha_b = ptr(self.alpha_linear.weight), ptr(self.alpha_linear.bias)
        mp.rgb_w, mp.rgb_b = ptr(self.rgb_linear.weight), ptr(self.rgb_linear.bias)
        return mp

    def packed_f16(self):
        params = list(self.parameters())
        key = tuple((p.data_ptr(), p._version) for p in params)
        self._f16_poll()
        if self._packed16 is not None and key == self._packed16_key:
            return self._packed16
        lib = _lib.load()
        n = lib.nerfail_mlp_f16_image_bytes(self.D, self.W, self._skip())
        if n == 0:
            raise NotImplementedError('unsupported NeRF shape D=%d W=%d' % (self.D, self.W))
        self.check_f16x3_range()
        keep = []
        mp = self._mlp_params(keep)
        buf = torch.empty((n,), dtype=torch.uint8, device=params[0].device)
        _lib.check(lib.nerfail_mlp_pack_f16(mp, _lib.dev(buf), _lib.stream()))
        self._packed16, self._packed16_key = buf, key
        return buf

    F16X3_MAX_WEIGHT = 60.0

    def check_f16x3_range(self, sync=False):
        self._f16_poll()
        ws = [p.detach() for n_, p in self.named_parameters() if n_.endswith('weight')]
        with torch.no_grad():
            m = torch.stack(torch._foreach_norm(ws, float('inf'))).max()
        if sync or not m.is_cuda or not getattr(self, '_f16_checked_once', False):
            self._f16_checked_once = True
            self._f16_verdict(float(m))
            return
        self._f16_poll(wait=True)
        host = getattr(self, '_f16_host', None)
        if host is None:
            host = self._f16_host = torch.empty((1,), dtype=torch.float32).pin_memory()
        host.copy_(m.reshape(1), non_blocking=True)
        ev = torch.cuda.Event()
        ev.record()
        self._f16_pending = ev

    def _f16_poll(self, wait=False):
        ev = getattr(self, '_f16_pending', None)
        if ev is None:
            return
        if wait:
            ev.synchronize()
        if ev.query():
            self._f16_pending = None
            self._f16_verdict(float(self._f16_host[0]))

    def _f16_verdict(self, m):
        if not m < self.F16X3_MAX_WEIGHT:
            raise ValueError("NeRF.precision = 'f16x3': max |weight| = %g is outside the range of the split-precision kernels "
                             "(|w| < %g); use precision = 'f32'" % (m, self.F16X3_MAX_WEIGHT))

    def forward(self, x):
        x = _lib.f32c(x, _cuda())
        assert x.shape[-1] == self.input_ch + self.input_ch_views
        flat = x.reshape(-1, x.shape[-1])
        out = torch.empty((flat.shape[0], 4), dtype=torch.float32, device=flat.device)
        _lib.check(_lib.load().nerfail_mlp_fwd_embedded_x3(_lib.dev(self.packed()), _lib.dev(self.packed_x3()), self.D, self.W,
                                                           self._skip(), _lib.dev(flat, 'x'), flat.shape[0], _lib.dev(out),
                                                           _lib.stream()))
        return out.reshape(x.shape[:-1] + (4,))


def _k4(K):
    return _lib.host_floats([K[0][0], K[1][1], K[0][2], K[1][2]])


def _c2w12(c2w):
    c = torch.as_tensor(c2w).detach().to('cpu', torch.float32)[:3, :4].reshape(-1).tolist()
    return _lib.host_floats(c)


def get_rays(H, W, K, c2w):
    dev = _cuda()
    rays_o = torch.empty((H, W, 3), dtype=torch.float32, device=dev)
    rays_d = torch.empty((H, W, 3), dtype=torch.float32, device=dev)
    _lib.check(_lib.load().nerfail_get_rays(int(H), int(W), _k4(K), _c2w12(c2w), _lib.dev(rays_o), _lib.dev(rays_d),
                                            _lib.stream()))
    return rays_o, rays_d


def get_rays_np(H, W, K, c2w):
    o, d = get_rays(H, W, K, c2w)
    return o.cpu().numpy(), d.cpu().numpy()


def ndc_rays(H, W, focal, near, rays_o, rays_d):
    raise NotImplementedError('ndc_rays (RH:179-196) is LLFF-only; every NeRFail config sets ndc=False (RN:250-252)')


_LINSPACE = {}


def linspace01(n, device):
    key = (int(n), str(device))
    if key not in _LINSPACE:
        _LINSPACE[key] = torch.linspace(0., 1., steps=int(n)).to(device)
    return _LINSPACE[key]


def sample_pdf(bins, weights, N_samples, det=False, pytest=False, u=None):
    dev = _cuda()
    bins = _lib.f32c(bins, dev)
    weights = _lib.f32c(weights, dev)
    lead = bins.shape[:-1]
    nb = bins.shape[-1]
    assert weights.shape[-1] == nb - 1
    b2, w2 = bins.reshape(-1, nb), weights.reshape(-1, nb - 1)
    R = b2.shape[0]
    if pytest:
        np.random.seed(0)
        if det:
            u = torch.Tensor(np.linspace(0., 1., N_samples)).to(dev)
        else:
            u = torch.Tensor(np.random.rand(*(list(lead) + [N_samples]))).to(dev)
    elif u is None:
        u = linspace01(N_samples, dev) if det else torch.rand(list(lead) + [N_samples], device=dev)
    u = _lib.f32c(u, dev)
    is_row = int(u.dim() == 1)
    if not is_row:
        u = u.reshape(R, N_samples)
    from . import ops
    out = torch.ops.nerfail_mi.sample_pdf(b2, w2, u)
    return out.reshape(tuple(lead) + (N_samples,))
```

Before: 917,700.

## Fold feature linear layer into view layer weights for x3 forward kernel

```diff
diff --git a/include/nerfail_hip.h b/include/nerfail_hip.h
--- a/include/nerfail_hip.h
+++ b/include/nerfail_hip.h
@@ -8,7 +8,7 @@
 extern "C" {
 #endif
 
-#define NERFAIL_ABI_VERSION 11
+#define NERFAIL_ABI_VERSION 12
 
 #define NERFAIL_OK 0
 #define NERFAIL_EINVAL 1
@@ -82,6 +82,16 @@
                                 float* raw, void* stream);
 int nerfail_mlp_fwd_rays_x3(const float* packed, const void* x3, int D, int W, int skip, const float* rays,
                             const float* z_vals, int64_t n_rays, int samples_per_ray, float* raw, float* acts, void* stream);
+
+size_t nerfail_mlp_packed_x3f_bytes(int D, int W, int skip);
+size_t nerfail_mlp_x3f_composed_floats(int D, int W, int skip);
+int nerfail_mlp_pack_x3f(const float* packed, int D, int W, int skip, void* x3f, void* stream);
+int nerfail_mlp_fwd_x3f(const float* packed, const void* x3f, int D, int W, int skip, const float* pts, const float* viewdirs,
+                        int64_t M, int samples_per_ray, float* raw, void* stream);
+int nerfail_mlp_fwd_embedded_x3f(const float* packed, const void* x3f, int D, int W, int skip, const float* x, int64_t M,
+                                 float* raw, void* stream);
+int nerfail_mlp_fwd_rays_x3f(const float* packed, const void* x3f, int D, int W, int skip, const float* rays,
+                             const float* z_vals, int64_t n_rays, int samples_per_ray, float* raw, float* acts, void* stream);
 
 size_t nerfail_mlp_f16_image_bytes(int D, int W, int skip);
 int nerfail_mlp_pack_f16(const nerfail_mlp_params* params_host, void* image, void* stream);
diff --git a/nerfail_amd/_lib.py b/nerfail_amd/_lib.py
--- a/nerfail_amd/_lib.py
+++ b/nerfail_amd/_lib.py
@@ -6,7 +6,7 @@
 _HERE = os.path.dirname(os.path.abspath(__file__))
 LIB_PATH = os.environ.get('NERFAIL_HIP_LIB') or os.path.join(_HERE, 'lib', 'libnerfail_hip.so')
 
-ABI_VERSION = 11
+ABI_VERSION = 12
 MAX_DEPTH = 16
 DW_BF16X3, DW_ACCUMULATE = 1, 2
 RAY_FLOATS = 11
@@ -52,6 +52,12 @@
     'nerfail_mlp_fwd_x3': (c_i, [c_p, c_p, c_i, c_i, c_i, c_p, c_p, c_i64, c_i, c_p, c_p]),
     'nerfail_mlp_fwd_embedded_x3': (c_i, [c_p, c_p, c_i, c_i, c_i, c_p, c_i64, c_p, c_p]),
     'nerfail_mlp_fwd_rays_x3': (c_i, [c_p, c_p, c_i, c_i, c_i, c_p, c_p, c_i64, c_i, c_p, c_p, c_p]),
+    'nerfail_mlp_packed_x3f_bytes': (ctypes.c_size_t, [c_i, c_i, c_i]),
+    'nerfail_mlp_x3f_composed_floats': (ctypes.c_size_t, [c_i, c_i, c_i]),
+    'nerfail_mlp_pack_x3f': (c_i, [c_p, c_i, c_i, c_i, c_p, c_p]),
+    'nerfail_mlp_fwd_x3f': (c_i, [c_p, c_p, c_i, c_i, c_i, c_p, c_p, c_i64, c_i, c_p, c_p]),
+    'nerfail_mlp_fwd_embedded_x3f': (c_i, [c_p, c_p, c_i, c_i, c_i, c_p, c_i64, c_p, c_p]),
+    'nerfail_mlp_fwd_rays_x3f': (c_i, [c_p, c_p, c_i, c_i, c_i, c_p, c_p, c_i64, c_i, c_p, c_p, c_p]),
     'nerfail_mlp_f16_image_bytes': (ctypes.c_size_t, [c_i, c_i, c_i]),
     'nerfail_mlp_pack_f16': (c_i, [ctypes.POINTER(MlpParams), c_p, c_p]),
     'nerfail_mlp_fwd_f16': (c_i, [c_p, c_p, c_i, c_i, c_i, c_p, c_p, c_i64, c_i, c_p, c_p]),
diff --git a/nerfail_amd/csrc/mlp.hip b/nerfail_amd/csrc/mlp.hip
--- a/nerfail_amd/csrc/mlp.hip
+++ b/nerfail_amd/csrc/mlp.hip
@@ -6,7 +6,10 @@
 bool mlp_x3_covers(const MlpLayout& L, int W);
 size_t mlp_x3_bytes(const MlpLayout& L, int W);
 int pack_mlp_x3(const float* packed, const MlpLayout& L, int W, void* out, hipStream_t s);
-int launch_mlp_x3(const MlpArgs& a, const void* img, int W, hipStream_t s);
+int launch_mlp_x3(const MlpArgs& a, const void* img, int W, bool fold, hipStream_t s);
+size_t mlp_x3f_bytes(const MlpLayout& L, int W);
+size_t mlp_x3f_composed_floats(const MlpLayout& L, int W);
+int pack_mlp_x3f(const float* packed, const MlpLayout& L, int W, void* out, hipStream_t s);
 
 template <int NT, bool TRAIN>
 __global__ __launch_bounds__(256, 1) void nerf_mlp_fwd_kernel(MlpArgs a) {
@@ -146,11 +149,11 @@
     return NERFAIL_OK;
 }
 
-static int launch_mlp_x3_or(const MlpArgs& a, const void* img, int W, hipStream_t s) {
+static int launch_mlp_x3_or(const char* fn, const MlpArgs& a, const void* img, int W, bool fold, hipStream_t s) {
     if (a.acts == nullptr && (g_fwd_select == 0 || g_fwd_select == 3)) {
         if (g_fwd_select == 3 || (img != nullptr && mlp_x3_covers(a.lay, W))) {
-            if (img == nullptr) { set_error("nerfail_mlp_fwd_x3: NERFAIL_FWD_KERNEL=x without a bf16x3 image"); return NERFAIL_EINVAL; }
-            return launch_mlp_x3(a, img, W, s);
+            if (img == nullptr) { set_error("%s: NERFAIL_FWD_KERNEL=x without a bf16x3 image", fn); return NERFAIL_EINVAL; }
+            return launch_mlp_x3(a, img, W, fold, s);
         }
     }
     return launch_mlp(a, W, s);
@@ -167,8 +170,9 @@
 }
 
 enum MlpInput { kInPts, kInEmbedded, kInRays };
+enum MlpSel { kF32, kX3, kX3Fold };
 #define MLP_REQUIRE(cond, msg) do { if (!(cond)) { set_error("%s: %s", fn, msg); return NERFAIL_EINVAL; } } while (0)
-static int mlp_fwd_entry(const char* fn, MlpInput form, const float* packed, bool use_x3, const void* x3, int D, int W, int skip,
+static int mlp_fwd_entry(const char* fn, MlpInput form, const float* packed, MlpSel sel, const void* x3, int D, int W, int skip,
                          const float* in0, const float* in1, int64_t M, int spr, float* raw, float* acts, bool need_acts, void* stream) {
     MLP_REQUIRE(M >= 0, form == kInRays ? "n_rays is negative" : "M is negative");
     MLP_REQUIRE(form == kInEmbedded || spr >= 1, "samples_per_ray must be positive");
@@ -182,18 +186,18 @@
     a.pts = form == kInPts ? in0 : nullptr; a.viewdirs = form == kInPts ? in1 : nullptr;
     a.xemb = form == kInEmbedded ? in0 : nullptr;
     a.rays = form == kInRays ? in0 : nullptr; a.z = form == kInRays ? in1 : nullptr;
-    return use_x3 ? launch_mlp_x3_or(a, x3, W, as_stream(stream)) : launch_mlp(a, W, as_stream(stream));
+    return sel != kF32 ? launch_mlp_x3_or(fn, a, x3, W, sel == kX3Fold, as_stream(stream)) : launch_mlp(a, W, as_stream(stream));
 }
 #undef MLP_REQUIRE
 
 extern "C" int nerfail_mlp_fwd(const float* packed, int D, int W, int skip, const float* pts, const float* viewdirs,
                                int64_t M, int samples_per_ray, float* raw, void* stream) {
-    return mlp_fwd_entry(__func__, kInPts, packed, false, nullptr, D, W, skip, pts, viewdirs, M, samples_per_ray, raw, nullptr, false, stream);
+    return mlp_fwd_entry(__func__, kInPts, packed, kF32, nullptr, D, W, skip, pts, viewdirs, M, samples_per_ray, raw, nullptr, false, stream);
 }
 
 extern "C" int nerfail_mlp_fwd_embedded(const float* packed, int D, int W, int skip, const float* x, int64_t M, float* raw,
                                         void* stream) {
-    return mlp_fwd_entry(__func__, kInEmbedded, packed, false, nullptr, D, W, skip, x, nullptr, M, 1, raw, nullptr, false, stream);
+    return mlp_fwd_entry(__func__, kInEmbedded, packed, kF32, nullptr, D, W, skip, x, nullptr, M, 1, raw, nullptr, false, stream);
 }
 
 extern "C" size_t nerfail_mlp_train_acts_floats(int D, int W, int64_t M) {
@@ -204,12 +208,12 @@
 
 extern "C" int nerfail_mlp_fwd_train(const float* packed, int D, int W, int skip, const float* pts, const float* viewdirs,
                                      int64_t M, int samples_per_ray, float* raw, float* acts, void* stream) {
-    return mlp_fwd_entry(__func__, kInPts, packed, false, nullptr, D, W, skip, pts, viewdirs, M, samples_per_ray, raw, acts, true, stream);
+    return mlp_fwd_entry(__func__, kInPts, packed, kF32, nullptr, D, W, skip, pts, viewdirs, M, samples_per_ray, raw, acts, true, stream);
 }
 
 extern "C" int nerfail_mlp_fwd_rays(const float* packed, int D, int W, int skip, const float* rays, const float* z_vals,
                                     int64_t n_rays, int samples_per_ray, float* raw, float* acts, void* stream) {
-    return mlp_fwd_entry(__func__, kInRays, packed, false, nullptr, D, W, skip, rays, z_vals, n_rays, samples_per_ray, raw, acts, false, stream);
+    return mlp_fwd_entry(__func__, kInRays, packed, kF32, nullptr, D, W, skip, rays, z_vals, n_rays, samples_per_ray, raw, acts, false, stream);
 }
 
 extern "C" size_t nerfail_mlp_packed_x3_bytes(int D, int W, int skip) {
@@ -226,15 +230,47 @@
 
 extern "C" int nerfail_mlp_fwd_x3(const float* packed, const void* x3, int D, int W, int skip, const float* pts,
                                   const float* viewdirs, int64_t M, int samples_per_ray, float* raw, void* stream) {
-    return mlp_fwd_entry(__func__, kInPts, packed, true, x3, D, W, skip, pts, viewdirs, M, samples_per_ray, raw, nullptr, false, stream);
+    return mlp_fwd_entry(__func__, kInPts, packed, kX3, x3, D, W, skip, pts, viewdirs, M, samples_per_ray, raw, nullptr, false, stream);
 }
 
 extern "C" int nerfail_mlp_fwd_embedded_x3(const float* packed, const void* x3, int D, int W, int skip, const float* x, int64_t M,
                                            float* raw, void* stream) {
-    return mlp_fwd_entry(__func__, kInEmbedded, packed, true, x3, D, W, skip, x, nullptr, M, 1, raw, nullptr, false, stream);
+    return mlp_fwd_entry(__func__, kInEmbedded, packed, kX3, x3, D, W, skip, x, nullptr, M, 1, raw, nullptr, false, stream);
 }
 
 extern "C" int nerfail_mlp_fwd_rays_x3(const float* packed, const void* x3, int D, int W, int skip, const float* rays,
                                        const float* z_vals, int64_t n_rays, int samples_per_ray, float* raw, float* acts, void* stream) {
-    return mlp_fwd_entry(__func__, kInRays, packed, true, x3, D, W, skip, rays, z_vals, n_rays, samples_per_ray, raw, acts, false, stream);
-}
+    return mlp_fwd_entry(__func__, kInRays, packed, kX3, x3, D, W, skip, rays, z_vals, n_rays, samples_per_ray, raw, acts, false, stream);
+}
+
+extern "C" size_t nerfail_mlp_packed_x3f_bytes(int D, int W, int skip) {
+    MlpLayout L;
+    return make_layout(D, W, skip, L) ? mlp_x3f_bytes(L, W) : 0;
+}
+
+extern "C" size_t nerfail_mlp_x3f_composed_floats(int D, int W, int skip) {
+    MlpLayout L;
+    return make_layout(D, W, skip, L) ? mlp_x3f_composed_floats(L, W) : 0;
+}
+
+extern "C" int nerfail_mlp_pack_x3f(const float* packed, int D, int W, int skip, void* out, void* stream) {
+    MlpLayout L;
+    NF_REQUIRE(make_layout(D, W, skip, L), "unsupported (D, W)");
+    NF_REQUIRE(packed != nullptr && out != nullptr, "NULL pointer");
+    return pack_mlp_x3f(packed, L, W, out, as_stream(stream));
+}
+
+extern "C" int nerfail_mlp_fwd_x3f(const float* packed, const void* x3f, int D, int W, int skip, const float* pts,
+                                   const float* viewdirs, int64_t M, int samples_per_ray, float* raw, void* stream) {
+    return mlp_fwd_entry(__func__, kInPts, packed, kX3Fold, x3f, D, W, skip, pts, viewdirs, M, samples_per_ray, raw, nullptr, false, stream);
+}
+
+extern "C" int nerfail_mlp_fwd_embedded_x3f(const float* packed, const void* x3f, int D, int W, int skip, const float* x, int64_t M,
+                                            float* raw, void* stream) {
+    return mlp_fwd_entry(__func__, kInEmbedded, packed, kX3Fold, x3f, D, W, skip, x, nullptr, M, 1, raw, nullptr, false, stream);
+}
+
+extern "C" int nerfail_mlp_fwd_rays_x3f(const float* packed, const void* x3f, int D, int W, int skip, const float* rays,
+                                        const float* z_vals, int64_t n_rays, int samples_per_ray, float* raw, float* acts, void* stream) {
+    return mlp_fwd_entry(__func__, kInRays, packed, kX3Fold, x3f, D, W, skip, rays, z_vals, n_rays, samples_per_ray, raw, acts, false, stream);
+}
diff --git a/nerfail_amd/csrc/mlp_layout.h b/nerfail_amd/csrc/mlp_layout.h
--- a/nerfail_amd/csrc/mlp_layout.h
+++ b/nerfail_amd/csrc/mlp_layout.h
@@ -16,9 +16,19 @@
     if (s == 3 * bands + 1) return h ? -1 : 2;
     return -1;
 }
-__host__ __device__ inline int acc_channel(int r, int h) { return (r & 3) + 8 * (r >> 2) + 4 * h; }
-
-__host__ __device__ inline int hidden_channel(int s, int h) { return 32 * (s / 16) + acc_channel(s % 16, h); }
+__host__ __device__ constexpr int acc_channel(int r, int h) { return (r & 3) + 8 * (r >> 2) + 4 * h; }
+
+__host__ __device__ constexpr int hidden_channel(int s, int h) { return 32 * (s / 16) + acc_channel(s % 16, h); }
+__host__ __device__ constexpr int hidden_half(int c) { return (c >> 2) & 1; }
+__host__ __device__ constexpr int hidden_step(int c) { return 16 * (c >> 5) + (c & 3) + 4 * ((c & 31) >> 3); }
+__host__ __device__ constexpr int bias_index(int c) { return 32 * (c >> 5) + 16 * hidden_half(c) + (hidden_step(c) & 15); }
+constexpr bool hidden_inverse_holds() {
+    for (int c = 0; c < 256; ++c)
+        if (hidden_channel(hidden_step(c), hidden_half(c)) != c || hidden_step(c) >= 128 || bias_index(c) >= 256 ||
+            32 * (bias_index(c) >> 5) + acc_channel(bias_index(c) & 15, (bias_index(c) >> 4) & 1) != c) return false;
+    return true;
+}
+static_assert(hidden_inverse_holds(), "hidden_step / hidden_half / bias_index invert hidden_channel / the bias order");
 __host__ __device__ inline int weight_column(int emb0, int h0, int dir0, int NT, int s, int h) {
     if (emb0 >= 0) {
         if (s < 4 * kEmbQuads) { const int c = enc_channel(s, h, 10); return c < 0 ? -1 : emb0 + c; }
diff --git a/nerfail_amd/csrc/mlp_x3.hip b/nerfail_amd/csrc/mlp_x3.hip
--- a/nerfail_amd/csrc/mlp_x3.hip
+++ b/nerfail_amd/csrc/mlp_x3.hip
@@ -45,6 +45,15 @@
     X.pieces = off;
     return off % X3Cfg::GP == 0;
 }
+static inline bool make_x3f_layout(const MlpLayout& L, int W, X3Layout& X) {
+    if (!make_x3_layout(L, W, X)) return false;
+    const unsigned feature = X.off[L.D + 1] - X.off[L.D];
+    X.off[L.D + 1] = X.off[L.D];
+    X.pieces -= feature;
+    return X.pieces % X3Cfg::GP == 0;
+}
+__host__ __device__ inline unsigned x3f_const_floats(const MlpLayout& L) { return L.total - L.b_off[0]; }
+static inline unsigned x3f_composed_floats(const MlpLayout& L) { return (unsigned)(L.NT / 2 * 32) * (L.NT * 32) + kPiece; }
 
 __device__ __forceinline__ unsigned cvt_bf2(float x0, float x1) {
     return __builtin_bit_cast(unsigned, __builtin_convertvector((f32x2){x0, x1}, bf16x2));
@@ -58,7 +67,8 @@
     MlpLayout L;
     X3Layout X;
 };
-__global__ void pack_x3_kernel(const float* __restrict__ packed, X3PackArgs p, u32x4* __restrict__ img) {
+template <bool FOLD>
+__global__ void pack_x3_kernel(const float* __restrict__ packed, X3PackArgs p, u32x4* __restrict__ img, const float* __restrict__ wc) {
     const long g = (long)blockIdx.x * blockDim.x + threadIdx.x;
     const long ts = g >> 6;
     const int lane = (int)(g & 63);
@@ -74,6 +84,10 @@
     const f32x4 q0 = *reinterpret_cast<const f32x4*>(w + (q * OT32) * kPiece);
     const f32x4 q1 = *reinterpret_cast<const f32x4*>(w + ((q + 2) * OT32) * kPiece);
     float x[8] = {q0[0], q0[1], q0[2], q0[3], q1[0], q1[1], q1[2], q1[3]};
+    if (FOLD && l == p.L.D + 1 && u < p.L.NT) {
+#pragma unroll
+        for (int j = 0; j < 8; ++j) x[j] = wc[row * (32 * p.L.NT) + 32 * u + 4 * lg + (j & 3) + 16 * (j >> 2)];
+    }
     u32x4 hi, mid, lo;
 #pragma unroll
     for (int k = 0; k < 4; ++k) {
@@ -88,6 +102,39 @@
     o[0] = hi;
     o[64] = mid;
     o[128] = lo;
+}
+
+__device__ __forceinline__ float x3f_weight(const float* __restrict__ packed, const MlpLayout& L, int l, int OT32, int i, int c) {
+    const int s = hidden_step(c), h = hidden_half(c);
+    return packed[L.w_off[l] + ((s >> 2) * OT32 + (i >> 5)) * kPiece + ((i & 31) + 32 * h) * 4 + (s & 3)];
+}
+__global__ void compose_x3f_kernel(const float* __restrict__ packed, MlpLayout L, float* __restrict__ cst, float* __restrict__ comp) {
+    const int W = 32 * L.NT, WV = W / 2, D = L.D;
+    const int nconst = (int)x3f_const_floats(L);
+    int t = (int)(blockIdx.x * blockDim.x + threadIdx.x);
+    if (t < WV * W) {
+        const int i = t / W, j = t % W;
+        double acc = 0.;
+        for (int m = 0; m < W; ++m)
+            acc += (double)x3f_weight(packed, L, D + 1, L.NT / 2, i, m) * (double)x3f_weight(packed, L, D, L.NT, m, j);
+        comp[t] = (float)acc;
+        return;
+    }
+    t -= WV * W;
+    if (t >= nconst + kPiece) return;
+    const int pos = t < nconst ? t % kPiece : t - nconst;
+    const bool in_bias = t < nconst && t / kPiece == D;
+    if (t < nconst && !in_bias) { cst[t] = packed[L.b_off[0] + t]; return; }
+    const int ch = in_bias ? 32 * (pos >> 5) + acc_channel(pos & 15, (pos >> 4) & 1) : pos;
+    float v = 0.f;
+    if (ch < WV && pos < (in_bias ? W : WV)) {
+        double acc = 0.;
+        for (int m = 0; m < W; ++m)
+            acc += (double)x3f_weight(packed, L, D + 1, L.NT / 2, ch, m) * (double)packed[L.b_off[D] + bias_index(m)];
+        acc += (double)packed[L.b_off[D + 1] + bias_index(ch)];
+        v = (float)acc;
+    }
+    (t < nconst ? cst[t] : comp[WV * W + pos]) = v;
 }
 
 struct X3Ring {
@@ -285,7 +332,7 @@
     }
 }
 
-template <int NT, int SKIP>
+template <int NT, int SKIP, bool FOLD>
 __global__ __launch_bounds__(256, 1) void nerf_mlp_fwd_x3_kernel(MlpArgs a, const void* img, int img_pieces) {
     static_assert(NT == X3Cfg::NT, "W = 256 only");
     using C = X3Cfg;
@@ -303,7 +350,7 @@
     const float* const park_rd = park_w + (c + 32 * (g & 1)) * 4 + (g >> 1) * 256;
     {
         const int n = (int)(L.total - L.b_off[0]);
-        const float* __restrict__ gm = a.packed + L.b_off[0];
+        const float* __restrict__ gm = FOLD ? static_cast<const float*>(img) + (long)img_pieces * kPiece : a.packed + L.b_off[0];
         for (int i = tid * 4; i < n; i += 1024) *reinterpret_cast<f32x4*>(cst + i) = *reinterpret_cast<const f32x4*>(gm + i);
     }
     __syncthreads();
@@ -346,7 +393,13 @@
             float emb[4 * kEmbQuads], demb[4 * kDirQuads];
             int hh = h;
             asm volatile("" : "+v"(hh));
-            encode_sample(a, s, hh, emb, demb);
+            if constexpr (FOLD) {
+                MlpArgs ar = a;
+                asm volatile("" : "+s"(ar.spr));
+                encode_sample(ar, s, hh, emb, demb);
+            } else {
+                encode_sample(a, s, hh, emb, demb);
+            }
 #pragma unroll
             for (int k = 0; k < kEmbQuads; ++k)
                 *reinterpret_cast<f32x4*>(park + k * 256) = (f32x4){emb[4 * k], emb[4 * k + 1], emb[4 * k + 2], emb[4 * k + 3]};
@@ -370,29 +423,44 @@
 
         float alpha[2] = {0.f, 0.f};
         auto layer = [&](f32x4 (&in)[OT][2], f32x4 (&out)[OT][2], int l, bool may_skip, bool may_be_last) __attribute__((always_inline)) {
-            if (may_be_last && l == L.D) {
+            if (!FOLD && may_be_last && l == L.D) {
                 x3_head<OT>(in, c_alpha + lane_off, alpha);
                 alpha[0] += c_alpha[NT * 32];
                 alpha[1] += c_alpha[NT * 32];
             }
             if (may_skip && l == L.skip + 1) x3_part<OT, kEmbQuads / 4, false>(st, out, b_park(0), no_hook);
+            int lb = l + 1;
+            if constexpr (FOLD) asm volatile("" : "+s"(lb));
             x3_part<OT, NT, true>(st, out, b_acc(in), [&](int u, int t, int k) {
-                if (u > 0) { bias_tile(in, l + 1, 2 * u - 2, 8, t, k); bias_tile(in, l + 1, 2 * u - 1, 9, t, k); }
-                if (u == NT - 1) { bias_tile(in, l + 1, 2 * u, 10, t, k); bias_tile(in, l + 1, 2 * u + 1, 11, t, k); }
+                if (u > 0) { bias_tile(in, lb, 2 * u - 2, 8, t, k); bias_tile(in, lb, 2 * u - 1, 9, t, k); }
+                if (u == NT - 1) { bias_tile(in, lb, 2 * u, 10, t, k); bias_tile(in, lb, 2 * u + 1, 11, t, k); }
             });
+            if (FOLD && may_be_last && l == L.D - 1) {
+                x3_head<OT>(out, c_alpha + lane_off, alpha);
+                alpha[0] += c_alpha[NT * 32];
+                alpha[1] += c_alpha[NT * 32];
+            }
         };
 #pragma unroll 1
         for (int l = 1; l < L.D; l += 2) {
-            layer(P, Q, l, SKIP == 1, false);
-            layer(Q, P, l + 1, SKIP == 2, true);
-        }
+            layer(P, Q, l, SKIP == 1, FOLD);
+            if (!FOLD || l + 1 < L.D) layer(Q, P, l + 1, SKIP == 2, !FOLD);
+        }
+        float rgb[2][3];
+        if constexpr (FOLD) {
+            x3_part<OTV, NT, true>(st, P, b_acc(Q), [&](int u, int t, int k) { bias_tile(P, 0, OTV + u, 2, t, k); });
+            x3_part<OTV, kDirQuads / 4, false>(st, P, b_park(kEmbQuads), no_hook);
+            x3_head3<OTV>(P, c_rgb + lane_off, OTV * 16, rgb);
+#pragma unroll
+            for (int t = 0; t < OTV; ++t) { bias_tile(P, 0, t, 0, 0, 10); bias_tile(P, 0, t, 0, 1, 11); }
+        } else {
         x3_part<OTV, NT, false>(st, Q, b_acc(P), [&](int u, int t, int k) {
             if (u > 0) { bias_tile(P, 0, 2 * u - 2, 2, t, k); bias_tile(P, 0, 2 * u - 1, 3, t, k); }
             if (u == NT - 1) { bias_tile(P, 0, 2 * u, 4, t, k); bias_tile(P, 0, 2 * u + 1, 5, t, k); }
         });
         x3_part<OTV, kDirQuads / 4, false>(st, Q, b_park(kEmbQuads), no_hook);
-        float rgb[2][3];
         x3_head3<OTV>(Q, c_rgb + lane_off, OTV * 16, rgb);
+        }
         const int n = g & 1;
         int je = 16 * n + c;
         asm volatile("" : "+v"(je));
@@ -416,25 +484,54 @@
     return mlp_x3_covers(L, W) && make_x3_layout(L, W, X) ? (size_t)X.pieces * kPiece * 4 : 0;
 }
 
+size_t mlp_x3f_composed_floats(const MlpLayout& L, int W) { return mlp_x3_covers(L, W) ? x3f_composed_floats(L) : 0; }
+
+size_t mlp_x3f_bytes(const MlpLayout& L, int W) {
+    X3Layout X;
+    if (!mlp_x3_covers(L, W) || !make_x3f_layout(L, W, X)) return 0;
+    return ((size_t)X.pieces * kPiece + x3f_const_floats(L) + x3f_composed_floats(L)) * 4;
+}
+
 int pack_mlp_x3(const float* packed, const MlpLayout& L, int W, void* out, hipStream_t s) {
     X3PackArgs p;
     p.L = L;
     if (!mlp_x3_covers(L, W) || !make_x3_layout(L, W, p.X)) { set_error("nerfail_mlp_pack_x3: shape not covered (W = 256, even D <= 8)"); return NERFAIL_EINVAL; }
     const long threads = (long)p.X.pieces / 3 * 64;
-    pack_x3_kernel<<<dim3((unsigned)((threads + 255) / 256)), dim3(256), 0, s>>>(packed, p, reinterpret_cast<u32x4*>(out));
+    pack_x3_kernel<false><<<dim3((unsigned)((threads + 255) / 256)), dim3(256), 0, s>>>(packed, p, reinterpret_cast<u32x4*>(out), nullptr);
     NF_LAUNCHED("pack_x3_kernel");
     return NERFAIL_OK;
 }
 
-int launch_mlp_x3(const MlpArgs& a, const void* img, int W, hipStream_t s) {
-    X3Layout X;
-    if (!mlp_x3_covers(a.lay, W) || !make_x3_layout(a.lay, W, X)) { set_error("nerf_mlp_fwd_x3_kernel: shape not covered (W = 256, even D <= 8)"); return NERFAIL_EINVAL; }
-    if (a.M >= (1L << 36)) { set_error("nerfail_mlp_fwd: M must be below 2^36 samples per call"); return NERFAIL_EINVAL; }
+int pack_mlp_x3f(const float* packed, const MlpLayout& L, int W, void* out, hipStream_t s) {
+    X3PackArgs p;
+    p.L = L;
+    if (!mlp_x3_covers(L, W) || !make_x3f_layout(L, W, p.X)) { set_error("nerfail_mlp_pack_x3f: shape not covered (W = 256, even D <= 8)"); return NERFAIL_EINVAL; }
+    float* const cst = static_cast<float*>(out) + (size_t)p.X.pieces * kPiece;
+    float* const comp = cst + x3f_const_floats(L);
+    const long cthreads = (long)(W / 2) * W + x3f_const_floats(L) + kPiece;
+    compose_x3f_kernel<<<dim3((unsigned)((cthreads + 255) / 256)), dim3(256), 0, s>>>(packed, L, cst, comp);
+    NF_LAUNCHED("compose_x3f_kernel");
+    const long threads = (long)p.X.pieces / 3 * 64;
+    pack_x3_kernel<true><<<dim3((unsigned)((threads + 255) / 256)), dim3(256), 0, s>>>(packed, p, reinterpret_cast<u32x4*>(out), comp);
+    NF_LAUNCHED("pack_x3_kernel");
+    return NERFAIL_OK;
+}
+
+template <bool FOLD>
+static void launch_x3(const MlpArgs& a, const void* img, int pieces, hipStream_t s) {
     const dim3 grid(mlp_grid_blocks((a.M + 31) / 32)), block(256);
     const int skip_layer = a.lay.skip >= 0 ? a.lay.skip + 1 : -1;
-    if (skip_layer < 0) nerf_mlp_fwd_x3_kernel<8, 0><<<grid, block, 0, s>>>(a, img, (int)X.pieces);
-    else if (skip_layer & 1) nerf_mlp_fwd_x3_kernel<8, 1><<<grid, block, 0, s>>>(a, img, (int)X.pieces);
-    else nerf_mlp_fwd_x3_kernel<8, 2><<<grid, block, 0, s>>>(a, img, (int)X.pieces);
+    if (skip_layer < 0) nerf_mlp_fwd_x3_kernel<8, 0, FOLD><<<grid, block, 0, s>>>(a, img, pieces);
+    else if (skip_layer & 1) nerf_mlp_fwd_x3_kernel<8, 1, FOLD><<<grid, block, 0, s>>>(a, img, pieces);
+    else nerf_mlp_fwd_x3_kernel<8, 2, FOLD><<<grid, block, 0, s>>>(a, img, pieces);
+}
+
+int launch_mlp_x3(const MlpArgs& a, const void* img, int W, bool fold, hipStream_t s) {
+    X3Layout X;
+    if (!mlp_x3_covers(a.lay, W) || !(fold ? make_x3f_layout(a.lay, W, X) : make_x3_layout(a.lay, W, X))) { set_error("nerf_mlp_fwd_x3_kernel: shape not covered (W = 256, even D <= 8)"); return NERFAIL_EINVAL; }
+    if (a.M >= (1L << 36)) { set_error("nerfail_mlp_fwd: M must be below 2^36 samples per call"); return NERFAIL_EINVAL; }
+    if (fold) launch_x3<true>(a, img, (int)X.pieces, s);
+    else launch_x3<false>(a, img, (int)X.pieces, s);
     NF_LAUNCHED("nerf_mlp_fwd_x3_kernel");
     return NERFAIL_OK;
 }
diff --git a/nerfail_amd/run_nerf.py b/nerfail_amd/run_nerf.py
--- a/nerfail_amd/run_nerf.py
+++ b/nerfail_amd/run_nerf.py
@@ -35,19 +35,22 @@
                                                    _lib.dev(pts, 'pts'), _lib.dev(viewdirs, 'viewdirs'), R * N, N,
                                                    _lib.dev(raw), _lib.stream()))
         return raw
-    _lib.check(_lib.load().nerfail_mlp_fwd_x3(_lib.dev(fn.packed()), _lib.dev(fn.packed_x3()), fn.D, fn.W, fn._skip(),
-                                              _lib.dev(pts, 'pts'), _lib.dev(viewdirs, 'viewdirs'), R * N, N, _lib.dev(raw),
-                                              _lib.stream()))
+    lib = _lib.load()
+    fold, img = fn.x3_image()
+    fwd = lib.nerfail_mlp_fwd_x3f if fold else lib.nerfail_mlp_fwd_x3
+    _lib.check(fwd(_lib.dev(fn.packed()), _lib.dev(img), fn.D, fn.W, fn._skip(), _lib.dev(pts, 'pts'),
+                   _lib.dev(viewdirs, 'viewdirs'), R * N, N, _lib.dev(raw), _lib.stream()))
     return raw
 
 
 def _mlp_rays(fn, rays, z_vals, acts=None):
     R, N = z_vals.shape
     raw = torch.empty((R, N, 4), dtype=torch.float32, device=z_vals.device)
-    x3 = fn.packed_x3() if acts is None else None
-    _lib.check(_lib.load().nerfail_mlp_fwd_rays_x3(_lib.dev(fn.packed()), _lib.dev(x3), fn.D, fn.W, fn._skip(),
-                                                   _lib.dev(rays, 'rays'), _lib.dev(z_vals, 'z_vals'), R, N, _lib.dev(raw),
-                                                   _lib.dev(acts), _lib.stream()))
+    lib = _lib.load()
+    fold, img = fn.x3_image() if acts is None else (False, None)
+    fwd = lib.nerfail_mlp_fwd_rays_x3f if fold else lib.nerfail_mlp_fwd_rays_x3
+    _lib.check(fwd(_lib.dev(fn.packed()), _lib.dev(img), fn.D, fn.W, fn._skip(), _lib.dev(rays, 'rays'),
+                   _lib.dev(z_vals, 'z_vals'), R, N, _lib.dev(raw), _lib.dev(acts), _lib.stream()))
     return raw
 
 
diff --git a/nerfail_amd/run_nerf_helpers.py b/nerfail_amd/run_nerf_helpers.py
--- a/nerfail_amd/run_nerf_helpers.py
+++ b/nerfail_amd/run_nerf_helpers.py
@@ -91,6 +91,8 @@
         self._packed16_key = None
         self._packed_x3 = None
         self._packed_x3_key = None
+        self._packed_x3f = None
+        self._packed_x3f_key = None
         self.precision = 'f32'
 
     def _skip(self):
@@ -133,6 +135,28 @@
             _lib.check(lib.nerfail_mlp_pack_x3(_lib.dev(f32), self.D, self.W, self._skip(), _lib.dev(buf), _lib.stream()))
         self._packed_x3, self._packed_x3_key = buf, key
         return buf
+
+    def packed_x3f(self):
+        f32 = self.packed()
+        params = list(self.parameters())
+        key = tuple((p.data_ptr(), p._version) for p in params)
+        if self._packed_x3f_key == key:
+            return self._packed_x3f
+        lib = _lib.load()
+        n = lib.nerfail_mlp_packed_x3f_bytes(self.D, self.W, self._skip())
+        buf = None
+        if n:
+            buf = torch.empty((n,), dtype=torch.uint8, device=f32.device)
+            _lib.check(lib.nerfail_mlp_pack_x3f(_lib.dev(f32), self.D, self.W, self._skip(), _lib.dev(buf), _lib.stream()))
+            composed = buf[n - 4 * lib.nerfail_mlp_x3f_composed_floats(self.D, self.W, self._skip()):].view(torch.float32)
+            if not bool(torch.isfinite(composed).all()):
+                buf = None
+        self._packed_x3f, self._packed_x3f_key = buf, key
+        return buf
+
+    def x3_image(self):
+        img = self.packed_x3f()
+        return (True, img) if img is not None else (False, self.packed_x3())
 
     def _mlp_params(self, keep):
         mp = _lib.MlpParams()
@@ -209,9 +233,11 @@
         assert x.shape[-1] == self.input_ch + self.input_ch_views
         flat = x.reshape(-1, x.shape[-1])
         out = torch.empty((flat.shape[0], 4), dtype=torch.float32, device=flat.device)
-        _lib.check(_lib.load().nerfail_mlp_fwd_embedded_x3(_lib.dev(self.packed()), _lib.dev(self.packed_x3()), self.D, self.W,
-                                                           self._skip(), _lib.dev(flat, 'x'), flat.shape[0], _lib.dev(out),
-                                                           _lib.stream()))
+        lib = _lib.load()
+        fold, img = self.x3_image()
+        fwd = lib.nerfail_mlp_fwd_embedded_x3f if fold else lib.nerfail_mlp_fwd_embedded_x3
+        _lib.check(fwd(_lib.dev(self.packed()), _lib.dev(img), self.D, self.W, self._skip(), _lib.dev(flat, 'x'), flat.shape[0],
+                       _lib.dev(out), _lib.stream()))
         return out.reshape(x.shape[:-1] + (4,))
 
 
```

After: 1.024 million, median of 6. +11.6%, better.
